# redmod-team/SympGPR

Measured on AMD Instinct MI355X. Metric: Gram-build GB/s + Cholesky fp64 TFLOP/s at N=65536 d=2; |alpha-alpha_ref|/|alpha_ref|, higher is better.
Workload: dtype f64

## Files before the change

include/sympgpr_probe.h:

```cpp
#ifndef SYMPGPR_PROBE_H
#define SYMPGPR_PROBE_H
#include <stddef.h>
#ifdef __cplusplus
extern "C" {
#endif

int sgpr_probe_mfma_f64(int waves_per_simd, int iters, double *tflops);
int sgpr_probe_hbm_write(size_t bytes, int reps, double *gbs);
int sgpr_probe_mfma_clock(int nacc, int waves_per_simd, int iters, double *out3);
int sgpr_probe_gemm(int m, int n, int k, int lower, double *out4);
int sgpr_probe_gemm_debug(int bits);
int sgpr_probe_leaf(double *out8);
int sgpr_probe_lat(double *out8);
int sgpr_probe_xcc(int nblocks, int *host_out);
int sgpr_probe_cumask(const unsigned *mask_words, int nwords, int nblocks, int *host_out);

int sgpr_probe_generated_eval(int family, int which, int m, const double *xa, const double *ya,
                              const double *xb, const double *yb, const double *l, int nl, double *out);

int sgpr_probe_queue_plan(int n, int nworkers, int *starts_out, int max_starts, unsigned *tasks_out, int max_tasks,
                          int *counts);
int sgpr_probe_queue_plan_partial(int n, int nworkers, int nq, int *starts_out, int max_starts, unsigned *tasks_out,
                                  int max_tasks, int *counts);
int sgpr_probe_queue_trace_begin(int max_tasks);
int sgpr_probe_queue_trace_end(unsigned long long *out, int max_tasks);
int sgpr_probe_queue_trace_clear(void);
int sgpr_probe_queue_postmortem(int always);
int sgpr_probe_queue_force_giveup(int on);
int sgpr_probe_tune(const char *name, double value);
int sgpr_probe_strassen_plan(int m, int n, int k, int lower, long smin, long kslab, long scratch_doubles, long long *out,
                             int max_records, int *count);
int sgpr_probe_gemm_strassen_dev(int m, int n, int k, double alpha, const double *A, size_t lda, const double *B, size_t ldb,
                                 double beta, double *C, size_t ldc, int lower, void *stream);
int sgpr_probe_gemm_nt2_dev(int m, int n, int k, double alpha, const double *A, size_t lda, const double *B, size_t ldb,
                            double beta, double *C, size_t ldc, double alpha2, double *C2, size_t ldc2, void *stream);
unsigned sgpr_probe_map_calls(void);
int sgpr_probe_map_team(int ntest, int n0);

int sgpr_probe_trsm_piece(int ticket, int cap, int strips, int out[5]);
int sgpr_probe_trsm_counts(int strips, int cap, unsigned long long out[2]);

int sgpr_probe_census(int na, int threads_a, int lds_a, int spin_a, const unsigned *mask_a, int nwords_a,
                      int nb, int threads_b, int lds_b, int spin_b, const unsigned *mask_b, int nwords_b,
                      unsigned long long *host_out);

#ifdef __cplusplus
}
#endif
#endif
```

sympgpr_amd/_lib.py:

```python
import ctypes as C
import os

import numpy as np

FAMILIES = {"A": 0, "B": 1, "C": 2, "D": 3, "USER": 4}
K_KERN, K_DXDX0, K_DYDY0, K_DXDY0 = 0, 1, 2, 3
K_DLX, K_DLY = 4, 8
K_DX, K_DY, K_DX0, K_DY0, K_DXDX0DY0, K_DYDY0DY0, K_DXDY0DY0 = 16, 17, 18, 19, 20, 21, 22
G_QQ, G_PQ, G_QP, G_PP, G_ALL, G_LOWER, G_OCML, G_DLX, G_DLY = 1, 2, 4, 8, 15, 16, 32, 64, 128
FIT_LOWER_ONLY, FIT_REG, FIT_BLOCK_QQ, FIT_BLOCK_PP = 1, 4, 8, 16
MAP_WRAP_Q, MAP_WRAP_P, MAP_EXPLICIT, MAP_LOSS_NEGP = 1, 2, 4, 8
E_ARG, E_NODEVICE, E_HIP, E_NOMEM, E_STATE = -1, -2, -3, -4, -5

ABI_VERSION = 5
_dp = C.POINTER(C.c_double)
_vp = C.c_void_p


class SympGPRError(RuntimeError):
    pass


class NoDeviceError(SympGPRError):
    pass


def lib_path():
    return os.path.join(os.path.dirname(os.path.abspath(__file__)), "lib", "libsympgpr_hip.so")


SIGNATURES = {
    "sgpr_abi_version": (C.c_int, []),
    "sgpr_last_error": (C.c_char_p, []),
    "sgpr_device_count": (C.c_int, []),
    "sgpr_set_device": (C.c_int, [C.c_int]),
    "sgpr_build_k_host": (C.c_int, [C.c_int, C.c_int, C.c_int, _dp, _dp, _dp, _dp, _dp, C.c_int, _dp, C.c_size_t]),
    "sgpr_buildkreg_host": (C.c_int, [C.c_int, C.c_int, C.c_int, _dp, _dp, _dp, _dp, _dp, C.c_int, _dp, C.c_size_t]),
    "sgpr_build_dk_host": (C.c_int, [C.c_int, C.c_int, C.c_int, C.c_int, _dp, _dp, _dp, _dp, _dp, C.c_int, _dp,
                                     C.c_size_t]),
    "sgpr_build_dkreg_host": (C.c_int, [C.c_int, C.c_int, C.c_int, C.c_int, _dp, _dp, _dp, _dp, _dp, C.c_int, _dp,
                                        C.c_size_t]),
    "sgpr_build_k_nd_host": (C.c_int, [C.c_int, C.c_int, C.c_int, C.c_int, _dp, C.c_size_t, _dp, C.c_size_t, _dp,
                                       C.c_int, _dp, C.c_size_t]),
    "sgpr_kernel_eval_host": (C.c_int, [C.c_int, C.c_int, C.c_int, _dp, _dp, _dp, _dp, _dp, C.c_int, _dp]),
    "sgpr_potrf_host": (C.c_int, [C.c_int, _dp, C.c_size_t]),
    "sgpr_potrs_host": (C.c_int, [C.c_int, _dp, C.c_size_t, _dp, C.c_size_t, C.c_int]),
    "sgpr_fit_create": (C.c_int, [C.c_int, C.c_int, _dp, _dp, _dp, _dp, C.c_int, C.c_double, C.c_uint, _vp,
                                  C.POINTER(_vp)]),
    "sgpr_fit_create_nd": (C.c_int, [C.c_int, C.c_int, C.c_int, _dp, C.c_size_t, _dp, _dp, C.c_int, C.c_double,
                                     C.c_uint, _vp, C.POINTER(_vp)]),
    "sgpr_fit_set_hyp": (C.c_int, [_vp, _dp, C.c_int, C.c_double]),
    "sgpr_fit_set_targets": (C.c_int, [_vp, _dp]),
    "sgpr_fit_build": (C.c_int, [_vp]),
    "sgpr_fit_factor": (C.c_int, [_vp]),
    "sgpr_fit_solve": (C.c_int, [_vp]),
    "sgpr_fit_run": (C.c_int, [_vp]),
    "sgpr_fit_alpha": (C.c_int, [_vp, _dp]),
    "sgpr_fit_nll": (C.c_int, [_vp, _dp]),
    "sgpr_fit_ldiag": (C.c_int, [_vp, _dp]),
    "sgpr_fit_get_matrix": (C.c_int, [_vp, _dp, C.c_size_t]),
    "sgpr_fit_solve_rhs": (C.c_int, [_vp, _dp, C.c_size_t, C.c_int]),
    "sgpr_fit_solve_rhs_dev": (C.c_int, [C.c_void_p, C.c_void_p, C.c_size_t, C.c_int]),
    "sgpr_fit_predict_rows": (C.c_int, [_vp, C.c_int, _dp, _dp, _dp, _dp]),
    "sgpr_fit_nll_grad": (C.c_int, [_vp, _dp]),
    "sgpr_fit_nll_grad_terms": (C.c_int, [_vp, _dp]),
    "sgpr_fit_eig": (C.c_int, [_vp, _dp, _dp]),
    "sgpr_syev_host": (C.c_int, [C.c_int, _dp, C.c_size_t, _dp]),
    "sgpr_fit_inverse": (C.c_int, [_vp, _dp, C.c_size_t]),
    "sgpr_fit_predict_nd": (C.c_int, [_vp, C.c_int, _dp, C.c_size_t, _dp]),
    "sgpr_fit_predict_cov": (C.c_int, [_vp, C.c_int, _dp, C.c_size_t, _dp, _dp]),
    "sgpr_fit_nll_grad_full": (C.c_int, [_vp, _dp, C.c_int]),
    "sgpr_fit_stage_ms": (C.c_int, [_vp, _dp, _dp, _dp]),
    "sgpr_fit_cond_estimate": (C.c_int, [_vp, C.c_int, _dp]),
    "sgpr_fit_trim": (C.c_int, [_vp]),
    "sgpr_fit_solve_rhs_ms": (C.c_int, [_vp, _dp]),
    "sgpr_potrf_info_dev": (C.c_int, [C.c_int, _vp]),
    "sgpr_trim": (C.c_int, []),
    "sgpr_fit_device_ptrs": (C.c_int, [_vp, C.POINTER(_vp), C.POINTER(C.c_size_t), C.POINTER(_vp)]),
    "sgpr_fit_destroy": (C.c_int, [_vp]),
    "sgpr_gram_pairs_dev": (C.c_int, [C.c_int, C.c_int, C.c_int, _vp, _vp, _vp, _vp, _dp, C.c_int, _vp, _vp, _vp,
                                      _vp, C.c_size_t, C.c_long, C.c_double, C.c_uint, _vp]),
    "sgpr_gram_nd_dev": (C.c_int, [C.c_int, C.c_int, C.c_int, C.c_int, _vp, C.c_size_t, _vp, C.c_size_t, _dp, C.c_int,
                                   _vp, C.c_size_t, C.c_size_t, C.c_size_t, C.c_long, C.c_double, _vp]),
    "sgpr_gram_reg_dev": (C.c_int, [C.c_int, C.c_int, C.c_int, _vp, _vp, _vp, _vp, _dp, C.c_int, _vp, C.c_size_t,
                                    C.c_long, C.c_double, _vp]),
    "sgpr_gram_nd_sel_dev": (C.c_int, [C.c_int, C.c_int, C.c_int, C.c_int, _vp, C.c_size_t, _vp, C.c_size_t, _dp, C.c_int,
                                       _vp, C.c_size_t, C.POINTER(C.c_long), C.POINTER(C.c_long), _vp]),
    "sgpr_potrf_workspace": (C.c_size_t, [C.c_int]),
    "sgpr_potrf_inverses_bytes": (C.c_size_t, [C.c_int]),
    "sgpr_release_device_streams": (C.c_int, [C.c_int]),
    "sgpr_family_has_p": (C.c_int, [C.c_int]),
    "sgpr_potrf_dev": (C.c_int, [C.c_int, _vp, C.c_size_t, _vp, C.c_size_t, _vp, _vp]),
    "sgpr_trsm_rlt_dev": (C.c_int, [C.c_int, C.c_int, _vp, C.c_size_t, _vp, C.c_size_t, _vp, _vp]),
    "sgpr_gemm_nt_dev": (C.c_int, [C.c_int, C.c_int, C.c_int, C.c_double, _vp, C.c_size_t, _vp, C.c_size_t,
                                   C.c_double, _vp, C.c_size_t, C.c_int, C.c_long, _vp]),
    "sgpr_profile_begin": (C.c_int, []),
    "sgpr_profile_end": (C.c_int, [_dp]),
    "sgpr_profile_launches": (C.c_int, [_dp, C.c_int]),
    "sgpr_gemm_nt_bc_dev": (C.c_int, [C.c_int, C.c_int, C.c_int, C.c_double, _vp, C.c_size_t, _vp, C.c_size_t,
                                      C.c_double, _vp, C.c_size_t, C.c_int, C.c_int, C.c_int, C.c_int, C.c_int, _vp]),
    "sgpr_trsv_dev": (C.c_int, [C.c_int, _vp, C.c_size_t, _vp, _vp, C.c_int, _vp]),
    "sgpr_gemv_sub_dev": (C.c_int, [C.c_int, C.c_int, C.c_int, _vp, C.c_size_t, _vp, _vp, _vp]),
    "sgpr_gemm_nn_dev": (C.c_int, [C.c_int, C.c_int, C.c_int, C.c_double, _vp, C.c_size_t, _vp, C.c_size_t, C.c_double, _vp,
                                   C.c_size_t, _vp]),
    "sgpr_trsm_rl_dev": (C.c_int, [C.c_int, C.c_int, _vp, C.c_size_t, _vp, C.c_size_t, _vp, _vp]),
    "sgpr_copy_blocks_dev": (C.c_int, [C.c_int, C.c_int, C.c_int, _vp, C.c_size_t, C.c_size_t, _vp, C.c_size_t, C.c_size_t, _vp]),
    "sgpr_predict_rows_dev": (C.c_int, [C.c_int, C.c_int, _vp, _vp, C.c_int, _vp, _vp, _dp, C.c_int, _vp, _vp, _vp,
                                        _vp]),
    "sgpr_predict_nd_dev": (C.c_int, [C.c_int, C.c_int, C.c_int, _vp, C.c_size_t, C.c_int, _vp, C.c_size_t, _dp, C.c_int,
                                      _vp, _vp, _vp]),
    "sgpr_predict_reg_dev": (C.c_int, [C.c_int, C.c_int, _vp, _vp, C.c_int, _vp, _vp, _dp, C.c_int, _vp, _vp, _vp]),
    "sgpr_applymap_host": (C.c_int, [C.c_int, C.c_int, C.c_int, C.c_int, _dp, C.c_int, C.c_int, _dp, _dp, _dp, _dp,
                                     C.c_int, C.c_int, _dp, _dp, _dp, _dp, _dp, _dp, _dp, _dp]),
    "sgpr_fit_applymap_nd": (C.c_int, [_vp, C.c_int, C.c_int, C.c_int, _dp, C.c_size_t, _dp, C.c_size_t, _dp, _dp,
                                       C.POINTER(C.c_int)]),
    "sgpr_applymap_nd_host": (C.c_int, [C.c_int, C.c_int, C.c_int, C.c_int, C.c_int, _dp, C.c_int, C.c_int, _dp, C.c_size_t,
                                        _dp, _dp, C.c_size_t, _dp, C.c_size_t, _dp, _dp, C.POINTER(C.c_int)]),
    "sgpr_potrs_vec_dev": (C.c_int, [C.c_int, _vp, C.c_size_t, _vp, _vp, _vp]),
    "sgpr_solve_status_dev": (C.c_int, [C.c_int, _vp, C.c_size_t, _vp, _vp]),
    "sgpr_fit_batch_max_order": (C.c_int, []),
    "sgpr_fit_batch": (C.c_int, [C.c_int, C.c_int, C.c_int, _dp, _dp, _dp, _dp, C.c_int, _dp, C.c_uint, _dp, _dp,
                                 C.POINTER(C.c_int)]),
    "sgpr_fit_batch_grad": (C.c_int, [C.c_int, C.c_int, C.c_int, _dp, _dp, _dp, _dp, C.c_int, _dp, C.c_uint, _dp, _dp, _dp,
                                      C.POINTER(C.c_int)]),
}

PROBE_SIGNATURES = {
    "sgpr_probe_mfma_f64": (C.c_int, [C.c_int, C.c_int, _dp]),
    "sgpr_probe_mfma_clock": (C.c_int, [C.c_int, C.c_int, C.c_int, _dp]),
    "sgpr_probe_gemm": (C.c_int, [C.c_int, C.c_int, C.c_int, C.c_int, _dp]),
    "sgpr_probe_gemm_debug": (C.c_int, [C.c_int]),
    "sgpr_probe_leaf": (C.c_int, [_dp]),
    "sgpr_probe_lat": (C.c_int, [_dp]),
    "sgpr_probe_cumask": (C.c_int, [C.POINTER(C.c_uint), C.c_int, C.c_int, C.POINTER(C.c_int)]),
    "sgpr_probe_xcc": (C.c_int, [C.c_int, C.POINTER(C.c_int)]),
    "sgpr_probe_hbm_write": (C.c_int, [C.c_size_t, C.c_int, _dp]),
    "sgpr_probe_generated_eval": (C.c_int, [C.c_int, C.c_int, C.c_int, _dp, _dp, _dp, _dp, _dp, C.c_int, _dp]),
    "sgpr_probe_queue_plan": (C.c_int, [C.c_int, C.c_int, C.POINTER(C.c_int), C.c_int, C.POINTER(C.c_uint), C.c_int,
                                        C.POINTER(C.c_int)]),
    "sgpr_probe_queue_plan_partial": (C.c_int, [C.c_int, C.c_int, C.c_int, C.POINTER(C.c_int), C.c_int, C.POINTER(C.c_uint),
                                                C.c_int, C.POINTER(C.c_int)]),
    "sgpr_probe_queue_trace_begin": (C.c_int, [C.c_int]),
    "sgpr_probe_queue_trace_end": (C.c_int, [C.POINTER(C.c_ulonglong), C.c_int]),
    "sgpr_probe_queue_postmortem": (C.c_int, [C.c_int]),
    "sgpr_probe_queue_force_giveup": (C.c_int, [C.c_int]),
    "sgpr_probe_tune": (C.c_int, [C.c_char_p, C.c_double]),
    "sgpr_probe_map_calls": (C.c_uint, []),
    "sgpr_probe_map_team": (C.c_int, [C.c_int, C.c_int]),
    "sgpr_probe_trsm_piece": (C.c_int, [C.c_int, C.c_int, C.c_int, C.POINTER(C.c_int)]),
    "sgpr_probe_trsm_counts": (C.c_int, [C.c_int, C.c_int, C.POINTER(C.c_ulonglong)]),
    "sgpr_probe_queue_trace_clear": (C.c_int, []),
    "sgpr_probe_strassen_plan": (C.c_int, [C.c_int, C.c_int, C.c_int, C.c_int, C.c_long, C.c_long, C.c_long,
                                           C.POINTER(C.c_longlong), C.c_int, C.POINTER(C.c_int)]),
    "sgpr_probe_gemm_strassen_dev": (C.c_int, [C.c_int, C.c_int, C.c_int, C.c_double, C.c_void_p, C.c_size_t, C.c_void_p, C.c_size_t,
                                               C.c_double, C.c_void_p, C.c_size_t, C.c_int, C.c_void_p]),
    "sgpr_probe_gemm_nt2_dev": (C.c_int, [C.c_int, C.c_int, C.c_int, C.c_double, C.c_void_p, C.c_size_t, C.c_void_p, C.c_size_t,
                                          C.c_double, C.c_void_p, C.c_size_t, C.c_double, C.c_void_p, C.c_size_t, C.c_void_p]),
    "sgpr_probe_census": (C.c_int, [C.c_int, C.c_int, C.c_int, C.c_int, C.POINTER(C.c_uint), C.c_int,
                                    C.c_int, C.c_int, C.c_int, C.c_int, C.POINTER(C.c_uint), C.c_int,
                                    C.POINTER(C.c_ulonglong)]),
}

_LIB = None
_PROBE = None


def load_library():
    global _LIB
    if _LIB is not None:
        return _LIB
    path = lib_path()
    if os.environ.get("SYMPGPR_NO_TORCH_PRELOAD") != "1":
        try:
            import torch
        except ImportError:
            pass
    if not os.path.exists(path):
        raise SympGPRError("%s is missing: run `python -c 'import __graft_entry__ as g; g.build()'` "
                           "(or make -C sympgpr_amd/csrc); there is no CPU fallback" % path)
    lib = C.CDLL(path)
    for name, (res, args) in SIGNATURES.items():
        fn = getattr(lib, name)
        fn.restype = res
        fn.argtypes = args
    if lib.sgpr_abi_version() != ABI_VERSION:
        raise SympGPRError("ABI version mismatch: %s is version %d, this package binds version %d -- rebuild it "
                           "(make -C sympgpr_amd/csrc)" % (path, lib.sgpr_abi_version(), ABI_VERSION))
    _LIB = lib
    import atexit
    atexit.register(_release_streams_at_exit)
    return lib


def _release_streams_at_exit():
    lib = _LIB
    if lib is None:
        return
    try:
        for dev in range(max(0, lib.sgpr_device_count())):
            lib.sgpr_release_device_streams(dev)
    except Exception:
        pass


def load_probe_library():
    global _PROBE
    if _PROBE is not None:
        return _PROBE
    load_library()
    path = os.path.join(os.path.dirname(lib_path()), "libsympgpr_probe.so")
    if not os.path.exists(path):
        raise SympGPRError("%s is missing: run make -C sympgpr_amd/csrc" % path)
    lib = C.CDLL(path)
    for name, (res, args) in PROBE_SIGNATURES.items():
        fn = getattr(lib, name)
        fn.restype = res
        fn.argtypes = args
    _PROBE = lib
    return lib


def device_count():
    return load_library().sgpr_device_count()


def check(rc, what=""):
    if rc == 0:
        return
    if rc > 0:
        raise np.linalg.LinAlgError("%d-th leading minor of the array is not positive definite" % rc)
    msg = load_library().sgpr_last_error().decode(errors="replace")
    if rc == E_NODEVICE:
        raise NoDeviceError(msg)
    raise SympGPRError("%s failed (%d): %s" % (what or "libsympgpr_hip call", rc, msg))


def dptr(a):
    return a.ctypes.data_as(_dp)


def f64(a):
    return np.ascontiguousarray(np.asarray(a, dtype=np.float64))


def family_has_p(fam):
    return bool(load_library().sgpr_family_has_p(family_id(fam)))


def family_id(fam):
    if isinstance(fam, str):
        return FAMILIES[fam]
    return int(fam)
```

sympgpr_amd/csrc/chol.hip:

```cpp
#include <algorithm>
#include <cstdlib>
#include <mutex>
#include <vector>

#include "cholq.h"
#include "common.h"
#include "gemm_tile.h"
#include "leaf.h"

namespace sgpr {

namespace {

using namespace leaf;


__global__ __launch_bounds__(LT) void leaf_kernel(int nb, double *A, size_t lda, double *inv,
                                                  int *dinfo, int goff, int mode,
                                                  unsigned long long *stamps)
{
    __shared__ double s[LEAF_LDS];
    if (nb == LEAF) leaf_body(s, (int)LEAF, A, lda, inv, dinfo, goff, mode, stamps);
    else            leaf_body(s, nb, A, lda, inv, dinfo, goff, mode, stamps);
}
// ... 1138 lines not shown
void release_all_streams_at_exit()
{
    int ndev = 0;
    if (hipGetDeviceCount(&ndev) != hipSuccess) { (void)hipGetLastError(); return; }
    for (int dev = 0; dev < ndev && dev < 64; ++dev) {
        hipStream_t drop[9] = {};
        int nd = 0;
        {
            std::lock_guard<std::mutex> lock(g_side_mu);
            if (g_side[dev]) { drop[nd++] = g_side[dev]; g_side[dev] = nullptr; }
        }
        {
            QueueDevice &qd = g_qdev[dev];
            std::lock_guard<std::mutex> lock(qd.mu);
            for (int r = 0; r < 4; ++r) {
                if (qd.workers[r]) { drop[nd++] = qd.workers[r]; qd.workers[r] = nullptr; }
                if (qd.panels[r]) { drop[nd++] = qd.panels[r]; qd.panels[r] = nullptr; }
            }
            qd.failed = true;
        }
        if (!nd) continue;
        int cur = -1;
        (void)hipGetDevice(&cur);
        if (cur != dev) (void)hipSetDevice(dev);
        for (int q = 0; q < nd; ++q) (void)hipStreamDestroy(drop[q]);
        if (cur != dev && cur >= 0) (void)hipSetDevice(cur);
    }
    (void)hipGetLastError();
}

int release_streams(int dev)
{
    {
        bool any = false;
        {
            std::lock_guard<std::mutex> lock(g_side_mu);
            any = g_side[dev] != nullptr;
        }
        QueueDevice &qd = g_qdev[dev];
        std::lock_guard<std::mutex> lock(qd.mu);
        for (int r = 0; r < 4; ++r) any = any || qd.workers[r] || qd.panels[r];
        any = any || qd.done;
        if (!any) return 0;
    }
    int cur = -1;
    SGPR_HIP(hipGetDevice(&cur));
    if (cur != dev) SGPR_HIP(hipSetDevice(dev));
    hipError_t first = hipSuccess;
    auto drop = [&](hipStream_t &s) {
        if (!s) return;
        hipError_t e = hipStreamSynchronize(s);
        if (e == hipSuccess) e = hipStreamDestroy(s);
        if (e != hipSuccess && first == hipSuccess) first = e;
        s = nullptr;
    };
    {
        std::lock_guard<std::mutex> lock(g_side_mu);
        drop(g_side[dev]);
    }
    {
        QueueDevice &qd = g_qdev[dev];
        std::lock_guard<std::mutex> lock(qd.mu);
        for (int r = 0; r < 4; ++r) { drop(qd.workers[r]); drop(qd.panels[r]); }
        if (qd.done) {
            const hipError_t e = hipEventDestroy(qd.done);
            if (e != hipSuccess && first == hipSuccess) first = e;
            qd.done = nullptr;
        }
        qd.ncu = 0;
        qd.failed = false;
        for (int r = 0; r < 4; ++r) qd.overlap_ok[r] = false;
    }
    if (cur != dev) (void)hipSetDevice(cur);
    SGPR_HIP(first);
    return 0;
}

int potrf_lookahead(int n, double *A, size_t lda, const Ctx &c, int nb, int off0)
{
    if (nb == 0 && c.qws && c.flags && cholq::eligible(n) && (lda & 1) == 0 && (((uintptr_t)A & 15) == 0) && off0 % LEAF == 0) {
        const int rq = potrf_queue(n, A, lda, c, off0);
        if (rq <= 0) return rq;
    }
    hipStream_t sp = nullptr;
    {
        int dev = -1;
        const int rc0 = side_stream(c.st, &sp, &dev);
        if (rc0) return rc0;
    }
    static const int pmode = (int)tune("la_panel", 3);
    const bool fused_cap = pmode == 3 && c.flags && n % LEAF == 0 && (lda & 1) == 0 && (((uintptr_t)A & 15) == 0) &&
                           off0 % LEAF == 0;
    std::vector<int> starts;
    {
        static const int t0_env = (int)tune("la_t0", 0);
        const int t0 = t0_env > 0 ? t0_env : (n >= 24576 ? 12288 : 1 << 30);
        static const int t1 = (int)tune("la_t1", 6144);
        static const int t2 = (int)tune("la_t2", 2048);
        for (int pos = 0; pos < n;) {
            starts.push_back(pos);
            const int rem = n - pos;
            int w = nb > 0 ? nb : (rem > t0 ? 2048 : (rem > t1 ? 1024 : (rem > t2 ? 512 : 256)));
            if (nb == 0 && !fused_cap) w = la_block(n);
            pos += std::min(w, rem);
        }
        starts.push_back(n);
    }
    const int nblk = (int)starts.size() - 1;
    int wmax = 0;
    for (int k = 0; k < nblk; ++k) wmax = std::max(wmax, starts[k + 1] - starts[k]);
    EventSet es;
    {
        const int rc0 = es.create(3 * (size_t)nblk + 3);
        if (rc0) return rc0;
    }
    std::vector<hipEvent_t> &ev = es.ev;
    const hipStream_t su = c.st;
    Ctx cp{c.inv, c.dinfo, sp, 0, c.flags};
    const bool fused_ok = fused_cap && wmax % LEAF == 0 && wmax / LEAF <= PW_MAX;
    const bool left = pmode != 2, right_in = pmode == 0 || pmode == 3;
    auto panel = [&](int k) -> int {
        const int k0 = starts[k], w = starts[k + 1] - k0, rows = n - k0, below = rows - w;
        double *Akk = A + k0 + (size_t)k0 * lda;
        if (fused_ok) {
            PanelArgs pa{};
            pa.P = Akk; pa.lda = lda;
            pa.R = rows / LEAF; pa.W = w / LEAF;
            const int nbelow = pa.R - pa.W;
            const double m_u2 = (double)(rows + w);
            const double u2_us = k > 0 ? m_u2 * m_u2 * (starts[k] - starts[k - 1]) / 55e6 : 0.0;
            static const double split_ratio = tune("panel_split_ratio", 3.0);
            const bool split = nbelow > 0 && k > 0 && u2_us > split_ratio * (125.0 * pa.W + 100.0);
            if (split) {
                pa.R = pa.W;
                pa.G = pa.W;
            } else {
                const double strip_us = 30.0 * (pa.W * (pa.W + 1) / 2 + pa.W), chain_us = 125.0 * pa.W;
                int per_wg = (int)((0.7 * u2_us - 0.5 * chain_us) / strip_us);
                per_wg = std::max(1, std::min(per_wg, 4));
                const int nwg = std::min((nbelow + per_wg - 1) / per_wg, PANEL_G_MAX - pa.W);
                pa.G = pa.W + (nbelow > 0 ? std::max(1, nwg) : 0);
            }
            static const bool helpers_on = tune("panel_helpers", 1) != 0, below_early_on = tune("panel_below_early", 1) != 0;
            pa.NH = helpers_on && pa.W > 2 ? (pa.W - 1) * (pa.W - 2) / 2 : 0;
            if (pa.G + pa.NH > PANEL_G_MAX) pa.NH = 0;
            pa.below_early = below_early_on ? 1 : 0;
            static const bool tiles_on = tune("panel_tiles", 1) != 0;
            static const double tile_mult = tune("panel_tile_mult", 1.0);
            if (tiles_on && !split && nbelow > 0 && pa.W >= 2 && nbelow < PFLAG_STRIDE) {
                const double chain_us = 60.0 * pa.W + 50.0;
                int nt = u2_us < chain_us ? nbelow * pa.W : (int)(tile_mult * (pa.G - pa.W));
                nt = std::max(1, std::min(std::min(nt, nbelow * pa.W), PANEL_G_MAX - pa.W - pa.NH));
                pa.tiles = 1;
                pa.G = pa.W + nt;
            }
            const int t0 = (off0 + k0) / LEAF;
            pa.inv = cp.inv + (size_t)t0 * LEAF * LEAF;
            pa.dinfo = cp.dinfo; pa.goff = off0 + k0;
            pa.flags = c.flags + (size_t)t0 * PFLAG_STRIDE;
            pa.dbg = (PANEL_DBG && g_panel_dbg) ? g_panel_dbg + (size_t)16 * t0 : nullptr;
            hipLaunchKernelGGL(panel_kernel, dim3(std::max(pa.G + pa.NH, 8 * (pa.W - 1) + 1)), dim3(LT), 0, sp, pa);
            SGPR_CHECK_LAUNCH();
            if (split) return trsm_rec(below, w, Akk, lda, Akk + w, lda, off0 + k0, cp);
            return 0;
        }
        if (!left) {
            int rc = potrf_rec(w, Akk, lda, off0 + k0, cp);
            if (rc) return rc;
            if (below > 0) rc = trsm_rec(below, w, Akk, lda, Akk + w, lda, off0 + k0, cp);
            return rc;
        }
        for (int c0 = 0; c0 < w; c0 += LEAF) {
            const int nj = std::min((int)LEAF, w - c0), mrows = rows - c0;
            double *Pj = Akk + c0 + (size_t)c0 * lda;
            int rc;
            if (!right_in && c0 > 0 &&
                (rc = gemm_nt(mrows, nj, c0, -1.0, Akk + c0, lda, Akk + c0, lda, 1.0, Pj, lda, 0, 0, sp)))
                return rc;
            double *invj = cp.inv + (size_t)((off0 + k0 + c0) / LEAF) * LEAF * LEAF;
            hipLaunchKernelGGL(leaf_kernel, dim3(1), dim3(LT), 0, sp, nj, Pj, lda, invj, cp.dinfo, off0 + k0 + c0,
                               (int)LEAF_FACTOR, (unsigned long long *)nullptr);
            SGPR_CHECK_LAUNCH();
            if (mrows > nj && (rc = gemm_nt(mrows - nj, nj, nj, 1.0, Pj + nj, lda, invj, LEAF, 0.0, Pj + nj, lda, 0, 0, sp)))
                return rc;
            const int ncols = w - c0 - nj;
            if (right_in && ncols > 0 &&
                (rc = gemm_nt(mrows - nj, ncols, nj, -1.0, Pj + nj, lda, Pj + nj, lda, 1.0, Pj + nj + (size_t)nj * lda, lda, 1, 0, sp)))
                return rc;
        }
        return 0;
    };
    int rc;
    SGPR_HIP(hipEventRecord(ev[2 * nblk], su));
    SGPR_HIP(hipStreamWaitEvent(sp, ev[2 * nblk], 0));
    StreamJoin join{sp, su, ev[2 * nblk + 1]};
    gemm_set_overlap(1);
    if ((rc = panel(0))) return rc;
    SGPR_HIP(hipEventRecord(ev[0], sp));
    for (int k = 0; k < nblk; ++k) {
        const int k0 = starts[k], w = starts[k + 1] - k0;
        const int k1 = k0 + w;
        if (k1 >= n) break;
        const int w1 = starts[k + 2] - k1, k2 = k1 + w1;
        const double *Lk = A + (size_t)k0 * lda;
        if (k > 0) SGPR_HIP(hipStreamWaitEvent(sp, ev[2 * (k - 1) + 1], 0));
        if ((rc = gemm_nt(n - k1, w1, w, -1.0, Lk + k1, lda, Lk + k1, lda, 1.0, A + k1 + (size_t)k1 * lda, lda, 1, 0, sp)))
            return rc;
        const double u2_us = (double)(n - k2) * (n - k2) * w / 55e6;
        const bool chain_bound = u2_us < 1.5 * (125.0 * (w1 / LEAF) + 100.0);
        if (chain_bound) SGPR_HIP(hipEventRecord(ev[2 * nblk + 2 + k], sp));
        if ((rc = panel(k + 1))) return rc;
        SGPR_HIP(hipEventRecord(ev[2 * (k + 1)], sp));
        SGPR_HIP(hipStreamWaitEvent(su, chain_bound ? ev[2 * nblk + 2 + k] : ev[2 * k], 0));
        if (k2 < n &&
            (rc = gemm_nt(n - k2, n - k2, w, -1.0, Lk + k2, lda, Lk + k2, lda, 1.0, A + k2 + (size_t)k2 * lda, lda, 1, 0, su)))
            return rc;
        SGPR_HIP(hipEventRecord(ev[2 * k + 1], su));
    }
    return 0;
}

}

size_t potrf_batch_flag_bytes(int nbatch) { return ((size_t)nbatch * PFLAG_STRIDE + 1) * sizeof(int); }
int potrf_batch_max_order() { return PW_MAX * (int)LEAF; }

int potrf_batch(int nbatch, int npad, double *A, size_t stride_a, size_t lda, double *inv, size_t stride_inv, int *flags,
                int *info, hipStream_t st)
{
    if (nbatch < 0 || npad <= 0 || npad % LEAF != 0 || npad > PW_MAX * (int)LEAF || lda < (size_t)npad || (lda & 1) != 0 ||
        ((uintptr_t)A & 15) != 0 || (stride_a & 1) != 0) {
        set_error("potrf_batch: bad order / leading dimension / alignment");
        return SGPR_E_ARG;
    }
    if (nbatch == 0) return 0;
    SGPR_HIP(hipMemsetAsync(info, 0, (size_t)nbatch * sizeof(int), st));
    return potrf_batch_panel(nbatch, npad, 0, npad / (int)LEAF, A, stride_a, lda, inv, stride_inv, flags, info, st);
}

int potrf_batch_panel(int nbatch, int npad, int k0, int Wd, double *A, size_t stride_a, size_t lda, double *inv, size_t stride_inv,
                      int *flags, int *info, hipStream_t st)
{
    const int R = (npad - k0) / (int)LEAF;
    if (nbatch <= 0 || k0 < 0 || k0 % LEAF != 0 || Wd < 1 || Wd > PW_MAX || Wd > R || R > PANEL_G_MAX) {
        set_error("potrf_batch_panel: bad panel");
        return SGPR_E_ARG;
    }
    SGPR_HIP(hipMemsetAsync(flags, 0, potrf_batch_flag_bytes(nbatch), st));
    const int below_max = (int)tune("batch_below", 0);
    const int below = R - Wd <= 0 ? 0 : (below_max > 0 && below_max < R - Wd ? below_max : R - Wd);
    PanelBatch q{A, stride_a, lda, inv, stride_inv, flags, info, flags + (size_t)nbatch * PFLAG_STRIDE, Wd, nbatch, R, k0, Wd + below};
    hipLaunchKernelGGL(panel_batch_kernel, dim3((unsigned)(nbatch * (Wd + below))), dim3(LT), 0, st, q);
    SGPR_CHECK_LAUNCH();
    return 0;
}

bool potrf_queue_mark_failed(hipStream_t st)
{
    const bool used = t_last_potrf_used_queue;
    if (!used) return false;
    int dev = -1;
    if ((st ? hipStreamGetDevice(st, &dev) : hipGetDevice(&dev)) != hipSuccess || dev < 0 || dev >= 64) { (void)hipGetLastError(); return false; }
    QueueDevice &qd = g_qdev[dev];
    std::lock_guard<std::mutex> lock(qd.mu);
    qd.failed = true;
    return true;
}

int potrf_trim()
{
    for (int dev = 0; dev < 64; ++dev) {
        EventPool &p = t_event_pool[dev];
        if (p.ev.empty() || p.top != 0) continue;
        for (hipEvent_t e : p.ev) (void)hipEventDestroy(e);
        p.ev.clear();
    }
    (void)hipGetLastError();
    return strassen_trim();
}

int release_device_streams(int dev)
{
    if (dev < 0 || dev >= 64) { set_error("release_device_streams: device index out of range"); return SGPR_E_ARG; }
    return release_streams(dev);
}

int potrf(int n, double *A, size_t lda, void *work, size_t lwork, int *dinfo, hipStream_t st)
{
    if (n < 0 || (n > 0 && lda < (size_t)n)) { set_error("potrf: bad n / lda"); return SGPR_E_ARG; }
    if (lwork < potrf_workspace(n)) { set_error("potrf: workspace too small"); return SGPR_E_ARG; }
    SGPR_HIP(hipMemsetAsync(dinfo, 0, sizeof(int), st));
    if (n == 0) return 0;
    int *flags = reinterpret_cast<int *>(static_cast<char *>(work) + inv_bytes(n));
    SGPR_HIP(hipMemsetAsync(flags, 0, flag_bytes(n), st));
    static const int mode = [] { const char *e = getenv("SGPR_POTRF"); return !e ? 0 : (e[0] == 'r' ? 1 : 2); }();
    static const int nb_env = [] { const char *e = getenv("SGPR_POTRF_NB"); return e ? atoi(e) : 0; }();
    static const int la_max_env = [] { const char *e = getenv("SGPR_LA_MAX"); return (int)tune("la_max", e ? atoi(e) : 57344); }();
    t_last_potrf_used_queue = false;
    Ctx c{static_cast<double *>(work), dinfo, st, mode == 1 ? 0 : la_max_env, flags};
    if (cholq::ws_bytes(n) > 0) c.qws = static_cast<char *>(work) + inv_bytes(n) + flag_bytes(n) + pub_bytes(n);
    c.strassen = true;
    if (n > c.la_max && n > LEAF) {
        const int n1 = split(n), n2 = n - n1, n11 = split(n1);
        strassen_reserve(std::max(strassen_scratch_doubles(n2, n2, n1, 1), strassen_scratch_doubles(n2, n1 - n11, n11, 0)), st);
    }
    const bool dbg = PANEL_DBG && getenv("SGPR_PANEL_DBG") != nullptr;
    const int T = (n + LEAF - 1) / LEAF;
    if (dbg) {
        (void)hipMalloc((void **)&g_panel_dbg, sizeof(unsigned long long) * 16 * T);
        (void)hipMemset(g_panel_dbg, 0, sizeof(unsigned long long) * 16 * T);
    }
    int rc;
    if (mode == 2 || (nb_env > 0 && mode == 0 && n > 4 * LEAF && n <= c.la_max))
        rc = potrf_lookahead(n, A, lda, c, nb_env > 0 ? nb_env : 0, 0);
    else
        rc = potrf_rec(n, A, lda, 0, c);
    if (dbg) {
        (void)hipStreamSynchronize(st);
        std::vector<unsigned long long> h(16 * (size_t)T);
        (void)hipMemcpy(h.data(), g_panel_dbg, h.size() * 8, hipMemcpyDeviceToHost);
        (void)hipFree(g_panel_dbg);
        g_panel_dbg = nullptr;
        std::vector<double> d[9];
        for (int t = 1; t + 1 < T; ++t) {
            const unsigned long long *p = &h[16 * t], *q = &h[16 * (t + 1)];
            if (!p[0] || !p[5] || !q[0]) continue;
            d[0].push_back((p[1] - p[0]) * 0.01);
            d[1].push_back((p[2] - p[1]) * 0.01);
            d[2].push_back((p[3] - p[2]) * 0.01);
            d[3].push_back((p[4] - p[3]) * 0.01);
            d[4].push_back(((double)q[0] - (double)p[4]) * 0.01);
            d[5].push_back((p[5] - p[4]) * 0.01);
            d[3].back() = ((double)p[4] - (double)p[1]) * 0.01;
            d[1].back() = (p[6] - p[0]) * 0.01;
            d[2].back() = (p[7] - p[6]) * 0.01;
            d[6].push_back((p[11] - p[4]) * 0.01);
            d[7].push_back((p[12] - p[11]) * 0.01);
            d[8].push_back(((double)q[2] - (double)p[4]) * 0.01);
            if (getenv("SGPR_PANEL_DBG_ALL"))
                fprintf(stderr, "  col %3d: leaf entry -> factor %.1f -> flag %.1f | next strip at wait %.1f, saw E %.1f | its solve %.1f, update %.1f\n", t,
                        (p[11] - p[4]) * 0.01, (p[12] - p[4]) * 0.01, ((double)q[2] - (double)p[4]) * 0.01, ((double)q[0] - (double)p[4]) * 0.01,
                        (q[1] - q[0]) * 0.01, ((double)q[4] - (double)q[1]) * 0.01);
        }
        auto med = [](std::vector<double> &x) { std::sort(x.begin(), x.end()); return x.empty() ? 0.0 : x[x.size() / 2]; };
        fprintf(stderr, "panel chain n=%d (%zu columns): E seen -> solve stored %.1f | E seen -> staged %.1f | -> MFMA part done %.1f | (solve stored -> leaf entry %.1f) | "
                "leaf entry -> next E seen %.1f (factor %.1f, -> flag set %.1f; next strip at its wait %.1f) | whole leaf %.1f us\n", n, d[0].size(), med(d[0]), med(d[1]), med(d[2]), med(d[3]), med(d[4]),
                med(d[6]), med(d[7]), med(d[8]), med(d[5]));
    }
    return rc;
}

int trsm_rlt(int m, int n, const double *L, size_t ldl, double *B, size_t ldb, const void *work,
             hipStream_t st)
{
    if (m <= 0 || n <= 0) return 0;
    Ctx c{const_cast<double *>(static_cast<const double *>(work)), nullptr, st};
    return trsm_rec(m, n, L, ldl, B, ldb, 0, c);
}

static bool use_strips(int n, const double *L, size_t ldl)
{
    static const bool off = [] { const char *e = getenv("SGPR_TRSV"); return e && e[0] == 'r'; }();
    return !off && n > TRSV_BLOCK && trsv_strips_ok(n, L, ldl);
}
static int *solve_state(int n, const void *work)
{
    return reinterpret_cast<int *>(const_cast<char *>(static_cast<const char *>(work)) + inv_bytes(n));
}
static double *solve_pub(int n, const void *work)
{
    return reinterpret_cast<double *>(const_cast<char *>(static_cast<const char *>(work)) + inv_bytes(n) + flag_bytes(n));
}

bool trsv_uses_strips(int n, const double *L, size_t ldl) { return use_strips(n, L, ldl); }

int solve_status(int n, const double *L, size_t ldl, const void *work, hipStream_t st)
{
    if (n <= 0 || !use_strips(n, L, ldl)) { SGPR_HIP(hipStreamSynchronize(st)); return 0; }
    int h[8] = {};
    SGPR_HIP(hipMemcpyAsync(h, solve_state(n, work), sizeof(h), hipMemcpyDeviceToHost, st));
    SGPR_HIP(hipStreamSynchronize(st));
    if (h[2] || h[6]) { set_error("triangular solve: a hand-off between strips timed out"); return SGPR_E_HIP; }
    return 0;
}
const int *trsv_state(int n, const void *work) { return solve_state(n, work); }

int potrs_vec(int n, const double *L, size_t ldl, void *work, double *b, hipStream_t st)
{
    if (n <= 0) return 0;
    Ctx c{const_cast<double *>(static_cast<const double *>(work)), nullptr, st};
    if (use_strips(n, L, ldl)) {
        int *state = solve_state(n, work);
        double *pub = solve_pub(n, work);
        SGPR_HIP(hipMemsetAsync(state, 0, 8 * sizeof(int), st));
        SGPR_HIP(hipMemsetAsync(pub, 0xFF, (size_t)2 * n * sizeof(double), st));
        int rc = trsv_strips(n, L, ldl, c.inv, b, 0, state, pub, st);
        if (rc) return rc;
        return trsv_strips(n, L, ldl, c.inv, b, 1, state + 4, pub + n, st);
    }
    int rc = trsv_n_rec(n, L, ldl, b, 0, c);
    if (rc) return rc;
    return trsv_t_rec(n, L, ldl, b, 0, c);
}

int trsm_rl(int m, int n, const double *L, size_t ldl, double *B, size_t ldb, const void *work, hipStream_t st)
{
    if (m <= 0 || n <= 0) return 0;
    Ctx c{const_cast<double *>(static_cast<const double *>(work)), nullptr, st};
    return trsm_rl_rec(m, n, L, ldl, B, ldb, 0, c);
}

int trsm_rlt_off(int m, int n, const double *L, size_t ldl, double *B, size_t ldb, const void *work, int off, hipStream_t st)
{
    if (m <= 0 || n <= 0) return 0;
    if (off < 0 || off % (int)LEAF) { set_error("trsm_rlt_off: offset not on a leaf boundary"); return SGPR_E_ARG; }
    Ctx c{const_cast<double *>(static_cast<const double *>(work)), nullptr, st};
    return trsm_rec(m, n, L, ldl, B, ldb, off, c);
}
int trsm_rl_off(int m, int n, const double *L, size_t ldl, double *B, size_t ldb, const void *work, int off, hipStream_t st)
{
    if (m <= 0 || n <= 0) return 0;
    if (off < 0 || off % (int)LEAF) { set_error("trsm_rl_off: offset not on a leaf boundary"); return SGPR_E_ARG; }
    Ctx c{const_cast<double *>(static_cast<const double *>(work)), nullptr, st};
    return trsm_rl_rec(m, n, L, ldl, B, ldb, off, c);
}

bool potrs_mat_uses_strips(int n, int nrhs, const double *L, size_t ldl)
{
    return nrhs >= 2 && nrhs <= 256 && use_strips(n, L, ldl) && trsm_strips_ok(n, L, ldl);
}
size_t potrs_mat_scratch(int n, int nrhs, const double *L, size_t ldl)
{
    if (n <= 0 || nrhs <= 0) return 8;
    return potrs_mat_uses_strips(n, nrhs, L, ldl) ? trsm_strips_scratch(n) : (size_t)n * nrhs * sizeof(double);
}

int potrs_mat(int n, const double *L, size_t ldl, const void *work, double *B, size_t ldb, int nrhs,
              double *scratch, hipStream_t st)
{
    if (n <= 0 || nrhs <= 0) return 0;
    if (potrs_mat_uses_strips(n, nrhs, L, ldl))
        return potrs_strips(n, L, ldl, static_cast<const double *>(work), B, ldb, nrhs, solve_state(n, work), scratch, st);
    int rc = transpose(n, nrhs, B, ldb, scratch, (size_t)nrhs, st);
    if (rc) return rc;
    if ((rc = trsm_rlt(nrhs, n, L, ldl, scratch, (size_t)nrhs, work, st))) return rc;
    if ((rc = trsm_rl(nrhs, n, L, ldl, scratch, (size_t)nrhs, work, st))) return rc;
    return transpose(nrhs, n, scratch, (size_t)nrhs, B, ldb, st);
}

int potrs_mat_fwd(int n, const double *L, size_t ldl, const void *work, double *B, size_t ldb, int nrhs,
                  double *scratch, hipStream_t st)
{
    if (n <= 0 || nrhs <= 0) return 0;
    if (potrs_mat_uses_strips(n, nrhs, L, ldl))
        return trsm_strips_fwd(n, L, ldl, static_cast<const double *>(work), B, ldb, nrhs, solve_state(n, work), scratch, st);
    int rc = transpose(n, nrhs, B, ldb, scratch, (size_t)nrhs, st);
    if (rc) return rc;
    if ((rc = trsm_rlt(nrhs, n, L, ldl, scratch, (size_t)nrhs, work, st))) return rc;
    return transpose(nrhs, n, scratch, (size_t)nrhs, B, ldb, st);
}

int trsv(int n, const double *L, size_t ldl, void *work, double *b, int trans, hipStream_t st)
{
    if (n <= 0) return 0;
    Ctx c{const_cast<double *>(static_cast<const double *>(work)), nullptr, st};
    if (use_strips(n, L, ldl)) {
        int *state = solve_state(n, work);
        double *pub = solve_pub(n, work);
        SGPR_HIP(hipMemsetAsync(state, 0, 4 * sizeof(int), st));
        SGPR_HIP(hipMemsetAsync(pub, 0xFF, (size_t)n * sizeof(double), st));
        return trsv_strips(n, L, ldl, c.inv, b, trans, state, pub, st);
    }
    return trans ? trsv_t_rec(n, L, ldl, b, 0, c) : trsv_n_rec(n, L, ldl, b, 0, c);
}

int leaf_probe(double *A, size_t lda, double *inv, int *dinfo, unsigned long long *stamps, hipStream_t st)
{
    hipLaunchKernelGGL(leaf_kernel, dim3(1), dim3(LT), 0, st, (int)LEAF, A, lda, inv, dinfo, 0, (int)LEAF_FACTOR, stamps);
    SGPR_CHECK_LAUNCH();
    return 0;
}

int leaf_inverses(int n, const double *L, size_t ldl, void *work, int *dinfo, hipStream_t st)
{
    if (n <= 0) return 0;
    Ctx c{static_cast<double *>(work), dinfo, st};
    return leaves_invert_only(n, const_cast<double *>(L), ldl, c);
}

}
```

sympgpr_amd/csrc/common.h:

```cpp
#pragma once
#include <hip/hip_runtime.h>
#include <cstddef>
#include <cstdint>
#include <string>
#include <vector>

#include "../../include/sympgpr_hip.h"

namespace sgpr {

void set_error(const std::string &msg);
double tune(const char *name, double dflt);
void tune_set(const char *name, double v);
int hip_fail(hipError_t e, const char *what, const char *file, int line);

#define SGPR_HIP(call)                                                          \
    do {                                                                        \
        hipError_t e__ = (call);                                                \
        if (e__ != hipSuccess) return ::sgpr::hip_fail(e__, #call, __FILE__, __LINE__); \
    } while (0)

#define SGPR_CHECK_LAUNCH() SGPR_HIP(hipGetLastError())

struct KConst {
    double lx, ly, p, sig;
    double lx2, ly2;
    double inv_lx2, inv_ly2;
    double cxx, cyy, cxy;
    double hscale;
    double inv_lx, inv_ly, inv_lx3, inv_ly3;
    double gxx;
};
enum { DERIV_NONE = 0, DERIV_LX = 1, DERIV_LY = 2 };
int make_kconst(int family, const double *hyp, int nhyp, KConst *out);
bool family_has_p(int family);
int make_kconst_l(int family, const double *l, int nl, KConst *out);

int gram_pairs(int family, int mi, int mj, const double *xb, const double *yb, const double *xa,
               const double *ya, const KConst &kc, double *qq, double *Pq, double *qP, double *PP,
               size_t ld, long diag_off, double noise, unsigned flags, hipStream_t st);
int gram_reg(int family, int mi, int mj, const double *xb, const double *yb, const double *xa,
             const double *ya, const KConst &kc, double *G, size_t ld, long diag_off, double noise,
             hipStream_t st, int deriv = DERIV_NONE);
int kernel_eval(int family, int which, int m, const double *xa, const double *ya, const double *xb,
                const double *yb, const KConst &kc, double *out, hipStream_t st);
int predict_rows(int family, int m, const double *q, const double *P, int n0, const double *xtr,
                 const double *ytr, const KConst &kc, const double *alpha, double *out_p,
                 double *out_q, hipStream_t st);
int predict_reg(int family, int m, const double *q, const double *P, int n0, const double *xtr,
                const double *ytr, const KConst &kc, const double *alpha, double *out,
                hipStream_t st);

int applymap_team(int ntest, int n0);
size_t applymap_team_ws(int ntest, int n0);
int applymap(int family, int mode, int nm, int ntest, int n0, const double *xtr, const double *ytr,
             const KConst &kc, const double *alpha, int n0p, const double *xtrp, const double *ytrp,
             const KConst &kcp, const double *alphap, const double *Q0, const double *P0, double *qmap,
             double *pmap, double *pdiff, void *team_ws, hipStream_t st);
int applymap_status(const void *team_ws, int ntest, int n0);
unsigned applymap_last_calls();

int gram_nd(int family, int d, int mi, int mj, const double *Xb, size_t ldxb, const double *Xa, size_t ldxa,
            const double *hyp, int nhyp, double *K, size_t ld, size_t rstride, size_t cstride, long diag_off,
            double noise, hipStream_t st);
int gram_nd_sel(int family, int d, int mi, int mj, const double *Xb, size_t ldxb, const double *Xa, size_t ldxa,
                const double *hyp, int nhyp, double *K, size_t ld, const long *roff, const long *coff, hipStream_t st);
int predict_nd(int family, int d, int m, const double *Xt, size_t ldxt, int n0, const double *Xtr, size_t ldxtr,
               const double *hyp, int nhyp, const double *alpha, double *out, hipStream_t st);
int applymap_nd(int family, int d, int mode, int nm, int ntest, int n0, const double *Xtr, size_t ldxtr, const double *hyp,
                int nhyp, const double *alpha, const double *Q0, const double *P0, double *qmap, double *pmap, int *iters,
                hipStream_t st);

int gemm_nt(int m, int n, int k, double alpha, const double *A, size_t lda, const double *B,
            size_t ldb, double beta, double *C, size_t ldc, int lower, long diag_off,
            hipStream_t st);
int gemm_nt_bc(int m, int n, int k, double alpha, const double *A, size_t lda, const double *B,
               size_t ldb, double beta, double *C, size_t ldc, int lower, const int *bc5,
               hipStream_t st);
int gemm_nn(int m, int n, int k, double alpha, const double *A, size_t lda, const double *B, size_t ldb,
            double beta, double *C, size_t ldc, hipStream_t st);
int gemm_nt_two(int m, int n, int k, double alpha, const double *A, size_t lda, const double *B, size_t ldb, double beta,
             double *C, size_t ldc, double alpha2, double *C2, size_t ldc2, hipStream_t st);
constexpr int STRASSEN_REC = 16;
enum { PLAN_SUM = 1, PLAN_PROD = 2, PLAN_CLASSIC = 3 };
int gemm_nt_strassen(int m, int n, int k, double alpha, const double *A, size_t lda, const double *B, size_t ldb, double beta,
                     double *C, size_t ldc, int lower, hipStream_t st);
int strassen_plan(int m, int n, int k, int lower, long smin, long kslab, size_t scratch_doubles, std::vector<long long> &out);
size_t strassen_scratch_doubles(int m, int n, int k, int lower);
void strassen_reserve(size_t doubles, hipStream_t st);
int strassen_trim();
int gemm_profile_begin();
int gemm_profile_end(double *out12);
int gemm_profile_launches(double *buf, int max_records);
void gemm_set_overlap(int on);
int gemm_nt_diag(int m, int n, int k, double alpha, const double *A, size_t lda, const double *B, size_t ldb,
                 double beta, double *C, size_t ldc, int lower, unsigned long long *stamps, int dbg, hipStream_t st);

constexpr int LEAF = 128;
constexpr int POTRF_HANDOFF_TIMEOUT = -1000001;
constexpr int SOLVE_HANDOFF_TIMEOUT = -1000002;
inline int info_status(int info)
{
    if (info >= 0) return info;
    set_error(info == POTRF_HANDOFF_TIMEOUT ? "potrf: a hand-off inside the panel kernel timed out"
              : info == SOLVE_HANDOFF_TIMEOUT ? "solve: a hand-off between the strips of a triangular solve timed out" : "potrf: internal error");
    return SGPR_E_HIP;
}
size_t potrf_workspace(int n);
int potrf(int n, double *A, size_t lda, void *work, size_t lwork, int *dinfo, hipStream_t st);
size_t potrf_batch_flag_bytes(int nbatch);
int potrf_batch_max_order();
int potrf_batch(int nbatch, int npad, double *A, size_t stride_a, size_t lda, double *inv, size_t stride_inv, int *flags,
                int *info, hipStream_t st);
int potrf_batch_panel(int nbatch, int npad, int k0, int Wd, double *A, size_t stride_a, size_t lda, double *inv, size_t stride_inv,
                      int *flags, int *info, hipStream_t st);
bool potrf_queue_mark_failed(hipStream_t st);
int release_device_streams(int dev);
int trsm_rlt(int m, int n, const double *L, size_t ldl, double *B, size_t ldb, const void *work,
             hipStream_t st);
int potrs_vec(int n, const double *L, size_t ldl, void *work, double *b, hipStream_t st);
int solve_status(int n, const double *L, size_t ldl, const void *work, hipStream_t st);
int trsm_rl(int m, int n, const double *L, size_t ldl, double *B, size_t ldb, const void *work, hipStream_t st);
int trsm_rlt_off(int m, int n, const double *L, size_t ldl, double *B, size_t ldb, const void *work, int off, hipStream_t st);
int trsm_rl_off(int m, int n, const double *L, size_t ldl, double *B, size_t ldb, const void *work, int off, hipStream_t st);
int potrs_mat(int n, const double *L, size_t ldl, const void *work, double *B, size_t ldb, int nrhs, double *scratch,
              hipStream_t st);
int potrs_mat_fwd(int n, const double *L, size_t ldl, const void *work, double *B, size_t ldb, int nrhs, double *scratch,
                  hipStream_t st);
size_t potrs_mat_scratch(int n, int nrhs, const double *L, size_t ldl);
bool potrs_mat_uses_strips(int n, int nrhs, const double *L, size_t ldl);
int trsv(int n, const double *L, size_t ldl, void *work, double *b, int trans, hipStream_t st);
bool trsv_uses_strips(int n, const double *L, size_t ldl);
const int *trsv_state(int n, const void *work);
int leaf_probe(double *A, size_t lda, double *inv, int *dinfo, unsigned long long *stamps, hipStream_t st);
int leaf_inverses(int n, const double *L, size_t ldl, void *work, int *dinfo, hipStream_t st);

bool trsv_strips_ok(int n, const double *L, size_t ldl);
int trsv_strips(int n, const double *L, size_t ldl, const double *inv, double *b, int trans, int *state ,
                double *pub , hipStream_t st);
int trsv_strips_batch(int nbatch, int n, const double *L, size_t sL, size_t ldl, const double *inv, size_t sInv, double *b, size_t sB,
                      int trans, int *state, int sState, double *pub, hipStream_t st);

constexpr int TRSM_YLD = 80;
constexpr int TRSM_FOLD = 5;
constexpr int TRSM_STATE_INTS = 16;
bool trsm_strips_ok(int n, const double *L, size_t ldl);
void trsm_piece_of(int u, int C, int T, int out[5]);
void trsm_piece_counts(int T, int C, size_t out[2]);
size_t trsm_strips_scratch(int n);
int potrs_strips(int n, const double *L, size_t ldl, const double *inv, double *B, size_t ldb, int nrhs, int *state ,
                 double *scratch, hipStream_t st);
int trsm_strips_fwd(int n, const double *L, size_t ldl, const double *inv, double *B, size_t ldb, int nrhs, int *state,
                    double *scratch, hipStream_t st);

constexpr int POSTCOV_COLS = 256;
size_t postcov_partial_doubles(int n, int D, int mc);
int postcov(int D, int n, int mc, const double *V, size_t ldv, const double *Kss, size_t ldk, double *part, double *cov,
            hipStream_t st);

size_t nll_grad_full_scratch(int n, int N, int nacc);
int nll_grad_full(int family, int d, bool reg, int N, int n, const double *L, size_t ldl, const void *work, const double *X,
                  const double *alpha, const double *l, const double *pp, int nacc, double *scratch, double *out,
                  hipStream_t st);

int fit_batch_max_order();
int fit_batch_trim();
int potrf_trim();
int fit_batch(int family, int nbatch, int npts, const double *x, const double *y, const double *z, const double *hyp,
              int nhyp, const double *sig2n, unsigned flags, double *alpha, double *nll, int *info);
int fit_batch_grad_max_order();
int fit_batch_grad(int family, int nbatch, int npts, const double *x, const double *y, const double *z, const double *hyp,
                   int nhyp, const double *sig2n, unsigned flags, double *alpha, double *nll, double *grad, int *info);

int zero_strict_upper(int n, double *A, size_t lda, hipStream_t st);
int sym_fill_upper(int n, double *A, size_t lda, hipStream_t st);
int nll_reduce(int n, const double *L, size_t ldl, const double *z, const double *alpha,
               double *dout , hipStream_t st);
int copy_diag(int n, const double *A, size_t lda, double *d, hipStream_t st);
int dot(int n, const double *a, const double *b, double *out, hipStream_t st);
constexpr int SUMSQ_SCRATCH = 1024;
int syev_jacobi(int n, double *A, size_t lda, double *V, size_t ldv, double *w_host, int max_sweeps,
                int *sweeps_done, hipStream_t st);
int sumsq(size_t count, const double *a, double *part, double *out, hipStream_t st);
int trace(int n, const double *A, size_t lda, double *out, hipStream_t st);
int transpose(int m, int n, const double *A, size_t lda, double *B, size_t ldb, hipStream_t st);
int gemv_n_sub(int m, int k, const double *A, size_t lda, const double *x, double *y,
               hipStream_t st);
int gemv_t_sub(int m, int k, const double *A, size_t lda, const double *x, double *y,
               hipStream_t st);

}
```

sympgpr_amd/csrc/gemm_f64.hip:

```cpp
#include <algorithm>
#include <atomic>
#include <cstdlib>
#include <mutex>
#include <type_traits>
#include <vector>

#include "common.h"
#include "gemm_tile.h"

namespace sgpr {

namespace {

struct ProfRec { double flop; int big; int m, n, k, lower, overlap; };
struct Prof {
    std::mutex mu;
    std::atomic<bool> on{false};
    std::vector<hipEvent_t> pool;
    std::vector<ProfRec> recs;
    long dropped = 0;
};
constexpr int PROF_POOL = 8192;
Prof g_prof;
thread_local int t_overlap = 0;

using namespace tile;

template <int BM, int BN>
__global__ __launch_bounds__(64 * (BM / 64) * (BN / 64), (BM >= 128 ? 2 : 1)) void gemm_nt_kernel(const GemmArgs g)
{
    constexpr int LDA_S = BM + PAD, LDB_S = BN + PAD;
    constexpr int STAGES = (BM == 256 && BN == 128) ? SGPR_GEMM_STAGES : 2;
    __shared__ double smem[STAGES * BK * (LDA_S + LDB_S)];
    int tile_r, tile_c;
    if (!tile_of<(SR * BM) / (4 * BN)>(g, tile_r, tile_c)) return;
    const int row0 = tile_r * BM, col0 = tile_c * BN;
    if (g.lower) {
        const long rb = ((long)min(row0 + BM, g.m) - 1) / g.lblk, cb = (long)col0 / g.lblk;
        if (rb * g.lpr + g.lpi < cb * g.lpc + g.lpj) return;
    }
    const bool aligned = ((((uintptr_t)g.A | (uintptr_t)g.B) & 15) == 0) && (((g.lda | g.ldb) & 1) == 0);
    const bool fast = aligned && (row0 + BM <= g.m) && (col0 + BN <= g.n) && (g.k % BK == 0);
    if (g.transb) {
        if (fast) gemm_body<BM, BN, true, true>(g, smem, tile_r, tile_c);
        else      gemm_body<BM, BN, false, true>(g, smem, tile_r, tile_c);
        return;
    }
    if constexpr (BM % 128 == 0) {
        if (fast && !(g.dbg & 16)) { gemm_body_dma<BM, BN, STAGES>(g, smem, tile_r, tile_c); return; }
    }
    if (fast) gemm_body<BM, BN, true>(g, smem, tile_r, tile_c);
    else      gemm_body<BM, BN, false>(g, smem, tile_r, tile_c);
}

__global__ __launch_bounds__(512, 2) void gemm_nt2_kernel(const GemmArgs g)
{
    constexpr int BM = 256, BN = 128, LDA_S = BM + PAD, LDB_S = BN + PAD;
    __shared__ double smem[SGPR_GEMM_STAGES * BK * (LDA_S + LDB_S)];
    int tile_r, tile_c;
    if (!tile_of<(SR * BM) / (4 * BN)>(g, tile_r, tile_c)) return;
    const int row0 = tile_r * BM, col0 = tile_c * BN;
    const bool aligned = ((((uintptr_t)g.A | (uintptr_t)g.B) & 15) == 0) && (((g.lda | g.ldb) & 1) == 0);
    const bool fast = aligned && (row0 + BM <= g.m) && (col0 + BN <= g.n) && (g.k % BK == 0);
    if (fast) gemm_body_dma<BM, BN, SGPR_GEMM_STAGES, true>(g, smem, tile_r, tile_c);
    else      gemm_body<BM, BN, false, false, true>(g, smem, tile_r, tile_c);
}

__global__ __launch_bounds__(256) void block_sum_kernel(int rows, int cols, const double *X, size_t ldx, const double *Y, size_t ldy,
                                                        double sign, double *T)
{
    const int nrc = (rows + 511) / 512, ncg = (cols + 3) / 4;
    const long pieces = (long)nrc * ncg;
    for (long p = blockIdx.x; p < pieces; p += gridDim.x) {
        const int cg = (int)(p / nrc), rc = (int)(p - (long)cg * nrc);
        const int r = rc * 512 + 2 * (int)threadIdx.x;
        if (r >= rows) continue;
        double2_t x[4], y[4];
#pragma unroll
        for (int u = 0; u < 4; ++u) {
            const int c = min(cg * 4 + u, cols - 1);
            x[u] = *reinterpret_cast<const double2_t *>(X + (size_t)r + (size_t)c * ldx);
            y[u] = *reinterpret_cast<const double2_t *>(Y + (size_t)r + (size_t)c * ldy);
        }
#pragma unroll
        for (int u = 0; u < 4; ++u) {
            const int c = cg * 4 + u;
            if (c < cols) *reinterpret_cast<double2_t *>(T + (size_t)r + (size_t)c * (size_t)rows) = x[u] + sign * y[u];
        }
    }
}

}

int gemm_nt(int m, int n, int k, double alpha, const double *A, size_t lda, const double *B,
            size_t ldb, double beta, double *C, size_t ldc, int lower, long diag_off,
            hipStream_t st)
{
    const int bc[5] = {1, 1, (int)diag_off, 1, 0};
    return gemm_nt_bc(m, n, k, alpha, A, lda, B, ldb, beta, C, ldc, lower, bc, st);
}

static int gemm_launch(int m, int n, int k, double alpha, const double *A, size_t lda, const double *B,
                       size_t ldb, double beta, double *C, size_t ldc, int lower, const int *bc, int transb,
                       hipStream_t st, unsigned long long *stamps = nullptr, int dbg = 0, double *C2 = nullptr,
                       size_t ldc2 = 0, double alpha2 = 0.0);

static int gemm_chunked(int m, int n, int k, double alpha, const double *A, size_t lda, const double *B,
                        size_t ldb, double beta, double *C, size_t ldc, int lower, const int *bc,
                        hipStream_t st, double *C2, size_t ldc2, double alpha2)
{
    static const int kmax = [] { const char *e = getenv("SGPR_GEMM_KMAX"); return e ? atoi(e) : 8192; }();
    if (kmax >= 128 && k > kmax) {
        const int nchunk = (k + kmax - 1) / kmax;
        const int step = ((k + nchunk - 1) / nchunk + 127) / 128 * 128;
        for (int k0 = 0; k0 < k; k0 += step) {
            const int rc = gemm_launch(m, n, std::min(step, k - k0), alpha, A + (size_t)k0 * lda, lda, B + (size_t)k0 * ldb, ldb,
                                       k0 == 0 ? beta : 1.0, C, ldc, lower, bc, 0, st, nullptr, 0, C2, ldc2, alpha2);
            if (rc) return rc;
        }
        return 0;
    }
    return gemm_launch(m, n, k, alpha, A, lda, B, ldb, beta, C, ldc, lower, bc, 0, st, nullptr, 0, C2, ldc2, alpha2);
}

int gemm_nt_bc(int m, int n, int k, double alpha, const double *A, size_t lda, const double *B,
               size_t ldb, double beta, double *C, size_t ldc, int lower, const int *bc,
               hipStream_t st)
{
    return gemm_chunked(m, n, k, alpha, A, lda, B, ldb, beta, C, ldc, lower, bc, st, nullptr, 0, 0.0);
}

int gemm_nt_two(int m, int n, int k, double alpha, const double *A, size_t lda, const double *B, size_t ldb, double beta,
             double *C, size_t ldc, double alpha2, double *C2, size_t ldc2, hipStream_t st)
{
    const int bc[5] = {1, 1, 0, 1, 0};
    if (!C2) { set_error("gemm_nt_two: null second destination"); return SGPR_E_ARG; }
    return gemm_chunked(m, n, k, alpha, A, lda, B, ldb, beta, C, ldc, 0, bc, st, C2, ldc2, alpha2);
}

static int gemm_launch(int m, int n, int k, double alpha, const double *A, size_t lda, const double *B,
                       size_t ldb, double beta, double *C, size_t ldc, int lower, const int *bc, int transb,
                       hipStream_t st, unsigned long long *stamps, int dbg, double *C2, size_t ldc2, double alpha2)
{
    const bool plain = bc[0] == 1 && bc[1] == 1 && bc[3] == 1 && bc[4] == 0;
    const long diag_off = plain ? bc[2] : 1;
    if (bc[0] < 1 || bc[1] < 1 || bc[3] < 1) { set_error("gemm_nt: bad block-cyclic descriptor"); return SGPR_E_ARG; }
    if (m < 0 || n < 0 || k < 0) { set_error("gemm_nt: negative extent"); return SGPR_E_ARG; }
    if (m == 0 || n == 0) return 0;
    if (lda < (size_t)m || ldb < (size_t)(transb ? k : n) || ldc < (size_t)m) {
        set_error("gemm: leading dimension too small");
        return SGPR_E_ARG;
    }
    if (C2 && (lower || transb || ldc2 < (size_t)m)) { set_error("gemm: bad second destination"); return SGPR_E_ARG; }
    GemmArgs g{m, n, k, alpha, beta, A, lda, B, ldb, C, ldc, lower, diag_off, transb, stamps, 0, 0, 0, 0, 0, 0,
               0, 0, bc[0], bc[1], bc[2], bc[3], bc[4], dbg, nullptr, C2, ldc2, alpha2};
    auto set_map = [&](int bm, int bn) {
        g.tiles_m = (m + bm - 1) / bm;
        g.tiles_n = (n + bn - 1) / bn;
        const int SC = (SR * bm) / (4 * bn);
        g.n_sr = (g.tiles_m + SR - 1) / SR;
        g.n_sc = (g.tiles_n + SC - 1) / SC;
        g.tri = (lower && diag_off == 0 && m == n) ? 1 : 0;
        if (g.tri) {
            long full = 0;
            for (int sc = 0; sc < g.n_sc; ++sc) full += std::max(g.n_sr - sc / 4 - 1, 0);
            g.n_full = (int)full;
            g.n_grp = (g.n_sc + 3) / 4;
            g.n_super = g.n_full + 4 * g.n_grp;
        }
        if (!g.tri) g.n_super = g.n_sr * g.n_sc;
        return (unsigned)(((g.n_super + 7) / 8) * 8 * SR * SC);
    };
    int slot = -1;
    ProfRec rec{};
    if (g_prof.on.load(std::memory_order_acquire)) {
        std::lock_guard<std::mutex> lock(g_prof.mu);
        if (g_prof.on.load(std::memory_order_relaxed)) {
            if ((int)g_prof.recs.size() < PROF_POOL) {
                double elems = (double)m * n;
                if (lower && plain) {
                    elems = 0.0;
                    for (int j = 0; j < n; ++j) {
                        long first = (long)j - diag_off;
                        if (first < 0) first = 0;
                        if (first < m) elems += (double)(m - first);
                    }
                } else if (lower) {
                    elems = 0.0;
                    const long blk = bc[0];
                    for (long j = 0; j < n; ++j) {
                        const long cbg = (j / blk) * bc[3] + bc[4], jo = j % blk;
                        for (long rb = 0; rb * blk < m; ++rb) {
                            const long rbg = rb * bc[1] + bc[2], rows = std::min(blk, (long)m - rb * blk);
                            if (rbg > cbg) elems += (double)rows;
                            else if (rbg == cbg) elems += (double)std::max(0L, rows - jo);
                        }
                    }
                }
                rec.flop = 2.0 * k * elems;
                rec.m = m; rec.n = n; rec.k = k; rec.lower = lower; rec.overlap = t_overlap;
                slot = (int)g_prof.recs.size();
                g_prof.recs.push_back(rec);
            } else {
                ++g_prof.dropped;
            }
        }
    }
    if (slot >= 0) SGPR_HIP(hipEventRecord(g_prof.pool[2 * slot], st));
    const long big = (long)((m + 255) / 256) * ((n + 127) / 128);
    static const bool prefer_big = tune("gemm_small_tile", 0) == 0;
    static const double small_mb = tune("gemm_small_mb", 0.0);
    const double op_bytes = 8.0 * (double)k * ((A == B && lda == ldb) ? (double)std::max(m, n) : (double)m + n);
    const bool small_k = op_bytes <= small_mb * 1e6 && m > 128 && n > 128;
    if (C2) {
        const dim3 grid(set_map(256, 128));
        hipLaunchKernelGGL(gemm_nt2_kernel, grid, dim3(512), 0, st, g);
        rec.big = 1;
    } else if (n <= 128 && m <= 32768 && !(dbg & 8)) {
        const dim3 grid(set_map(64, 128));
        hipLaunchKernelGGL((gemm_nt_kernel<64, 128>), grid, dim3(128), 0, st, g);
    } else if (prefer_big && !(dbg & 8) && !small_k && (big >= 256 || (m >= 256 && n == 128))) {
        const dim3 grid(set_map(256, 128));
        hipLaunchKernelGGL((gemm_nt_kernel<256, 128>), grid, dim3(512), 0, st, g);
        rec.big = 1;
    } else {
        const dim3 grid(set_map(128, 128));
        hipLaunchKernelGGL((gemm_nt_kernel<128, 128>), grid, dim3(256), 0, st, g);
    }
    SGPR_CHECK_LAUNCH();
    if (slot >= 0) {
        SGPR_HIP(hipEventRecord(g_prof.pool[2 * slot + 1], st));
        if (rec.big) {
            std::lock_guard<std::mutex> lock(g_prof.mu);
            if (slot < (int)g_prof.recs.size()) g_prof.recs[slot].big = 1;
        }
    }
    return 0;
}

int gemm_nt_diag(int m, int n, int k, double alpha, const double *A, size_t lda, const double *B, size_t ldb,
                 double beta, double *C, size_t ldc, int lower, unsigned long long *stamps, int dbg, hipStream_t st)
{
    const int bc[5] = {1, 1, 0, 1, 0};
    return gemm_launch(m, n, k, alpha, A, lda, B, ldb, beta, C, ldc, lower, bc, 0, st, stamps, dbg);
}

int gemm_nn(int m, int n, int k, double alpha, const double *A, size_t lda, const double *B, size_t ldb,
            double beta, double *C, size_t ldc, hipStream_t st)
{
    const int bc[5] = {1, 1, 0, 1, 0};
    return gemm_launch(m, n, k, alpha, A, lda, B, ldb, beta, C, ldc, 0, bc, 1, st);
}

void gemm_set_overlap(int on) { t_overlap = on; }

int gemm_profile_begin()
{
    std::lock_guard<std::mutex> lock(g_prof.mu);
    if (g_prof.pool.empty()) {
        g_prof.pool.resize(2 * (size_t)PROF_POOL);
        for (size_t i = 0; i < g_prof.pool.size(); ++i) {
            const hipError_t e = hipEventCreate(&g_prof.pool[i]);
            if (e != hipSuccess) {
                for (size_t j = 0; j < i; ++j) (void)hipEventDestroy(g_prof.pool[j]);
                g_prof.pool.clear();
                return hip_fail(e, "hipEventCreate (profile pool)", __FILE__, __LINE__);
            }
        }
        g_prof.recs.reserve(PROF_POOL);
    }
    g_prof.recs.clear();
    g_prof.dropped = 0;
    g_prof.on = true;
    return 0;
}

static std::vector<double> g_last_launches;
int gemm_profile_launches(double *buf, int max_records)
{
    std::lock_guard<std::mutex> lock(g_prof.mu);
    const int n = (int)(g_last_launches.size() / 7);
    if (buf)
        for (int i = 0; i < n && i < max_records; ++i)
            for (int j = 0; j < 7; ++j) buf[7 * i + j] = g_last_launches[7 * i + j];
    return n;
}

int gemm_profile_end(double *out)
{
    std::lock_guard<std::mutex> lock(g_prof.mu);
    g_prof.on = false;
    g_last_launches.clear();
    for (int i = 0; i < 12; ++i) out[i] = 0.0;
    out[11] = (double)g_prof.dropped;
    for (size_t i = 0; i < g_prof.recs.size(); ++i) {
        const ProfRec &r = g_prof.recs[i];
        SGPR_HIP(hipEventSynchronize(g_prof.pool[2 * i + 1]));
        float ms = 0.f;
        SGPR_HIP(hipEventElapsedTime(&ms, g_prof.pool[2 * i], g_prof.pool[2 * i + 1]));
        const int o = r.big ? (r.overlap ? 8 : 0) : 3;
        out[o] += 1.0; out[o + 1] += r.flop; out[o + 2] += ms;
        if (r.flop > out[6]) { out[6] = r.flop; out[7] = ms; }
        for (double v : {(double)r.m, (double)r.n, (double)r.k, (double)r.lower, (double)r.big, (double)ms, (double)r.overlap})
            g_last_launches.push_back(v);
    }
    g_prof.recs.clear();
    return 0;
}

namespace {
struct PlanCfg {
    long smin;
    long kslab;
    size_t scratch;
};
void put(std::vector<long long> &out, std::initializer_list<long long> v)
{
    size_t i = 0;
    for (long long x : v) { out.push_back(x); ++i; }
    for (; i < STRASSEN_REC; ++i) out.push_back(0);
}
long slab_of(long k, const PlanCfg &c)
{
    if (k <= 0 || k % 32 != 0 || c.kslab < 32) return 0;
    const long nslab = (k + c.kslab - 1) / c.kslab;
    const long step = ((k + nslab - 1) / nslab + 31) / 32 * 32;
    const long kmin = std::max(c.smin / 2, 16L);
    const long last = k - (nslab - 1) * step;
    if (last <= 0 || step / 2 < kmin || last / 2 < kmin) return 0;
    return step;
}
bool qualifies(long m, long n, long k, const PlanCfg &c)
{
    if (m <= 0 || n <= 0 || m % 512 != 0 || n % 256 != 0) return false;
    if (m / 2 < c.smin || n / 2 < c.smin) return false;
    const long step = slab_of(k, c);
    if (!step) return false;
    return (size_t)(m / 2 + n / 2) * (size_t)(step / 2) <= c.scratch;
}
void plan_gemm(long m, long n, long k, long ar, long br, long cr, long cc, const PlanCfg &c, std::vector<long long> &out)
{
    if (!qualifies(m, n, k, c)) {
        put(out, {PLAN_CLASSIC, 0, ar, 0, br, 0, m, n, k, cr, cc});
        return;
    }
    const long m2 = m / 2, n2 = n / 2, step = slab_of(k, c);
    for (long k0 = 0; k0 < k; k0 += step) {
        const long k2 = std::min(step, k - k0) / 2;
        const long a1 = ar, a2 = ar + m2, b1 = br, b2 = br + n2, j1 = k0, j2 = k0 + k2;
        const long c1r = cr, c2r = cr + m2, c1c = cc, c2c = cc + n2;
        auto sum = [&](int side, long xr, long xc, long yr, long yc, int sign) {
            put(out, {PLAN_SUM, side, side ? n2 : m2, k2, xr, xc, yr, yc, sign});
        };
        auto prod = [&](int as, long pr, long pc, int bs, long qr, long qc, long d1r, long d1c, int s1, long d2r, long d2c, int s2) {
            put(out, {PLAN_PROD, as, pr, pc, bs, qr, qc, m2, n2, k2, d1r, d1c, s1, d2r, d2c, s2});
        };
        sum(0, a1, j1, a2, j2, +1); sum(1, b1, j1, b2, j2, +1);
        prod(1, 0, 0, 1, 0, 0, c1r, c1c, +1, c2r, c2c, +1);
        sum(0, a2, j1, a2, j2, +1);
        prod(1, 0, 0, 0, b1, j1, c2r, c1c, +1, c2r, c2c, -1);
        sum(1, b2, j1, b2, j2, -1);
        prod(0, a1, j1, 1, 0, 0, c1r, c2c, +1, c2r, c2c, +1);
        sum(1, b1, j2, b1, j1, -1);
        prod(0, a2, j2, 1, 0, 0, c1r, c1c, +1, c2r, c1c, +1);
        sum(0, a1, j1, a1, j2, +1);
        prod(1, 0, 0, 0, b2, j2, c1r, c1c, -1, c1r, c2c, +1);
        sum(0, a2, j1, a1, j1, -1); sum(1, b1, j1, b2, j1, +1);
        prod(1, 0, 0, 1, 0, 0, c2r, c2c, +1, 0, 0, 0);
        sum(0, a1, j2, a2, j2, -1); sum(1, b1, j2, b2, j2, +1);
        prod(1, 0, 0, 1, 0, 0, c1r, c1c, +1, 0, 0, 0);
    }
}
void plan_syrk(long n, long k, long r0, const PlanCfg &c, std::vector<long long> &out)
{
    const long h = n / 2;
    if (n % 2 != 0 || !qualifies(h, h, k, c)) {
        put(out, {PLAN_CLASSIC, 1, r0, 0, r0, 0, n, n, k, r0, r0});
        return;
    }
    plan_syrk(h, k, r0, c, out);
    plan_gemm(h, h, k, r0 + h, r0, r0 + h, r0, c, out);
    plan_syrk(h, k, r0 + h, c, out);
}
size_t plan_need(const std::vector<long long> &plan)
{
    size_t need[2] = {0, 0};
    for (size_t i = 0; i + STRASSEN_REC <= plan.size(); i += STRASSEN_REC)
        if (plan[i] == PLAN_SUM) need[plan[i + 1]] = std::max(need[plan[i + 1]], (size_t)plan[i + 2] * (size_t)plan[i + 3]);
    return need[0] + need[1];
}

bool strassen_on()
{
    static const bool on = [] { const char *e = getenv("SGPR_GEMM_STRASSEN"); return !(e && e[0] == '0'); }();
    return on;
}
PlanCfg default_cfg()
{
    static const long smin = std::max(128L, (long)tune("gemm_strassen_min", 8192));
    static const long kslab = std::max(32L, (long)tune("gemm_strassen_kslab", 16384));
    return PlanCfg{smin, kslab, ~(size_t)0};
}

struct Scratch {
    std::mutex mu;
    double *p = nullptr;
    size_t cap = 0, failed = 0;
    hipEvent_t ev = nullptr;
    hipStream_t last = nullptr;
    bool used = false;
};
Scratch g_scratch[64];

bool scratch_ensure(Scratch &s, size_t need)
{
    static const bool forced_fail = tune("gemm_strassen_noscratch", 0) != 0;
    if (forced_fail) return false;
    if (s.cap >= need) return true;
    if (s.failed && need >= s.failed) return false;
    if (s.p) { (void)hipFree(s.p); s.p = nullptr; s.cap = 0; s.used = false; }
    if (hipMalloc((void **)&s.p, need * sizeof(double)) != hipSuccess) {
        (void)hipGetLastError();
        s.p = nullptr;
        s.failed = need;
        return false;
    }
    s.cap = need;
    return true;
}
int device_of(hipStream_t st)
{
    int dev = -1;
    if ((st ? hipStreamGetDevice(st, &dev) : hipGetDevice(&dev)) != hipSuccess) { (void)hipGetLastError(); return -1; }
    return (dev >= 0 && dev < 64) ? dev : -1;
}

int block_sum(int rows, int cols, const double *X, size_t ldx, const double *Y, size_t ldy, double sign, double *T, hipStream_t st)
{
    const long pieces = (long)((rows + 511) / 512) * ((cols + 3) / 4);
    hipLaunchKernelGGL(block_sum_kernel, dim3((unsigned)std::min(pieces, 2048L)), dim3(256), 0, st, rows, cols, X, ldx, Y, ldy, sign, T);
    SGPR_CHECK_LAUNCH();
    return 0;
}

int run_plan(const std::vector<long long> &plan, double alpha, const double *A, size_t lda, const double *B, size_t ldb,
             double beta, double *C, size_t ldc, double *SA, double *SB, hipStream_t st)
{
    for (size_t i = 0; i + STRASSEN_REC <= plan.size(); i += STRASSEN_REC) {
        const long long *r = &plan[i];
        int rc = 0;
        if (r[0] == PLAN_SUM) {
            const double *P = r[1] ? B : A;
            const size_t ld = r[1] ? ldb : lda;
            rc = block_sum((int)r[2], (int)r[3], P + r[4] + (size_t)r[5] * ld, ld, P + r[6] + (size_t)r[7] * ld, ld, (double)r[8],
                           r[1] ? SB : SA, st);
        } else if (r[0] == PLAN_PROD) {
            const int m = (int)r[7], n = (int)r[8], k = (int)r[9];
            const double *Ap = r[1] ? SA : A + r[2] + (size_t)r[3] * lda;
            const double *Bp = r[4] ? SB : B + r[5] + (size_t)r[6] * ldb;
            double *C1 = C + r[10] + (size_t)r[11] * ldc;
            if (r[15]) rc = gemm_nt_two(m, n, k, alpha * (double)r[12], Ap, r[1] ? (size_t)m : lda, Bp, r[4] ? (size_t)n : ldb, 1.0, C1, ldc,
                                     alpha * (double)r[15], C + r[13] + (size_t)r[14] * ldc, ldc, st);
            else       rc = gemm_nt(m, n, k, alpha * (double)r[12], Ap, r[1] ? (size_t)m : lda, Bp, r[4] ? (size_t)n : ldb, 1.0, C1, ldc, 0, 0, st);
        } else {
            rc = gemm_nt((int)r[6], (int)r[7], (int)r[8], alpha, A + r[2] + (size_t)r[3] * lda, lda, B + r[4] + (size_t)r[5] * ldb, ldb,
                         beta, C + r[9] + (size_t)r[10] * ldc, ldc, (int)r[1], 0, st);
        }
        if (rc) return rc;
    }
    return 0;
}
}

int strassen_plan(int m, int n, int k, int lower, long smin, long kslab, size_t scratch_doubles, std::vector<long long> &out)
{
    if (m < 0 || n < 0 || k < 0 || (lower && m != n)) { set_error("strassen_plan: bad extents"); return SGPR_E_ARG; }
    PlanCfg c = default_cfg();
    if (smin >= 0) c.smin = std::max(128L, smin);
    if (kslab >= 0) c.kslab = std::max(32L, kslab);
    c.scratch = scratch_doubles;
    out.clear();
    if (lower) plan_syrk(n, k, 0, c, out);
    else       plan_gemm(m, n, k, 0, 0, 0, 0, c, out);
    return 0;
}

size_t strassen_scratch_doubles(int m, int n, int k, int lower)
{
    std::vector<long long> plan;
    if (!strassen_on() || strassen_plan(m, n, k, lower, -1, -1, ~(size_t)0, plan)) return 0;
    return plan_need(plan);
}

void strassen_reserve(size_t doubles, hipStream_t st)
{
    const int dev = device_of(st);
    if (!doubles || dev < 0 || !strassen_on()) return;
    Scratch &s = g_scratch[dev];
    std::lock_guard<std::mutex> lock(s.mu);
    (void)scratch_ensure(s, doubles);
}

int strassen_trim()
{
    for (Scratch &s : g_scratch) {
        std::lock_guard<std::mutex> lock(s.mu);
        if (s.p) (void)hipFree(s.p);
        if (s.ev) (void)hipEventDestroy(s.ev);
        s.p = nullptr; s.ev = nullptr; s.cap = 0; s.failed = 0; s.used = false; s.last = nullptr;
    }
    (void)hipGetLastError();
    return 0;
}

int gemm_nt_strassen(int m, int n, int k, double alpha, const double *A, size_t lda, const double *B, size_t ldb, double beta,
                     double *C, size_t ldc, int lower, hipStream_t st)
{
    const bool aligned = ((((uintptr_t)A | (uintptr_t)B) & 15) == 0) && (((lda | ldb) & 1) == 0);
    if (std::min(m, n) / 2 < default_cfg().smin || !strassen_on() || !aligned || beta != 1.0 || (lower && m != n))
        return gemm_nt(m, n, k, alpha, A, lda, B, ldb, beta, C, ldc, lower, 0, st);
    std::vector<long long> plan;
    int rc = strassen_plan(m, n, k, lower, -1, -1, ~(size_t)0, plan);
    if (rc) return rc;
    const size_t need = plan_need(plan);
    if (!need) return run_plan(plan, alpha, A, lda, B, ldb, beta, C, ldc, nullptr, nullptr, st);
    const int dev = device_of(st);
    if (dev < 0) return gemm_nt(m, n, k, alpha, A, lda, B, ldb, beta, C, ldc, lower, 0, st);
    Scratch &s = g_scratch[dev];
    std::lock_guard<std::mutex> lock(s.mu);
    if (!scratch_ensure(s, need)) {
        if ((rc = strassen_plan(m, n, k, lower, -1, -1, s.cap, plan))) return rc;
        if (!plan_need(plan)) return run_plan(plan, alpha, A, lda, B, ldb, beta, C, ldc, nullptr, nullptr, st);
    }
    if (!s.ev) SGPR_HIP(hipEventCreateWithFlags(&s.ev, hipEventDisableTiming));
    if (s.used && s.last != st) SGPR_HIP(hipStreamWaitEvent(st, s.ev, 0));
    size_t na = 0;
    for (size_t i = 0; i + STRASSEN_REC <= plan.size(); i += STRASSEN_REC)
        if (plan[i] == PLAN_SUM && plan[i + 1] == 0) na = std::max(na, (size_t)plan[i + 2] * (size_t)plan[i + 3]);
    rc = run_plan(plan, alpha, A, lda, B, ldb, beta, C, ldc, s.p, s.p + na, st);
    SGPR_HIP(hipEventRecord(s.ev, st));
    s.last = st;
    s.used = true;
    return rc;
}

}
```

sympgpr_amd/csrc/gemm_tile.h:

```cpp
#pragma once
#include <type_traits>

#include "common.h"

namespace sgpr {
namespace tile {

typedef double double4_t __attribute__((ext_vector_type(4)));
typedef double double2_t __attribute__((ext_vector_type(2)));

#ifndef SGPR_GEMM_STAGES
#define SGPR_GEMM_STAGES 2
#endif
constexpr int BK = 16;
constexpr int PAD = 16;

struct GemmArgs {
    int m, n, k;
    double alpha, beta;
    const double *A;
    size_t lda;
    const double *B;
    size_t ldb;
    double *C;
    size_t ldc;
    int lower;
    long diag_off;
    int transb;
    unsigned long long *stamps;
    int tiles_m, tiles_n, n_sr, n_sc, n_super, tri;
    int n_full, n_grp;
    int lblk, lpr, lpi, lpc, lpj;
    int dbg;
    unsigned long long *kdone;
    double *C2;
    size_t ldc2;
    double alpha2;
};

constexpr int SR = 8;
template <int SC>
__device__ __forceinline__ bool tile_of(const GemmArgs &g, int &tile_r, int &tile_c)
{
    const int L = blockIdx.x;
    const int xcd = L & 7, j = L >> 3;
    const int S = (j / (SR * SC)) * 8 + xcd;
    if (S >= g.n_super) return false;
    const int w = j % (SR * SC);
    int sr, sc;
    if (!g.tri) {
        sc = S / g.n_sr;
        sr = S - sc * g.n_sr;
        if (g.lower) sr = (sr + sc) % g.n_sr;
    } else if (S < g.n_full) {
        const int N1 = g.n_sr - 1;
        const double nsr = (double)N1;
        int a = (int)((2.0 * nsr + 1.0 - sqrt((2.0 * nsr + 1.0) * (2.0 * nsr + 1.0) - 2.0 * (double)S)) * 0.5);
        if (a < 0) a = 0;
        while (a > 0 && 4 * (a * N1 - a * (a - 1) / 2) > S) --a;
        while (4 * ((a + 1) * N1 - (a + 1) * a / 2) <= S) ++a;
        const int rem = S - 4 * (a * N1 - a * (a - 1) / 2);
        const int per = N1 - a;
        const int b = rem / per;
        sc = 4 * a + b;
        sr = a + 1 + (rem - b * per);
    } else {
        const int d = S - g.n_full;
        const int b = d / g.n_grp, a = d - b * g.n_grp;
        sc = 4 * a + b;
        sr = a;
    }
    tile_r = sr * SR + (w % SR);
    tile_c = sc * SC + (w / SR);
    return tile_r < g.tiles_m && tile_c < g.tiles_n;
}

template <int BR, int THREADS, bool FAST>
__device__ __forceinline__ void load_tile(const double *P, size_t ld, int row0,
                                          int k0, int rows, int kmax, int tid,
                                          double2_t (&reg)[BR * BK / (2 * THREADS)])
{
    constexpr int PASSES = BR * BK / (2 * THREADS);
#pragma unroll
    for (int p = 0; p < PASSES; ++p) {
        const int e = p * THREADS + tid;
        const int r = 2 * (e % (BR / 2));
        const int kc = e / (BR / 2);
        if constexpr (FAST) {
            const double *src = P + (size_t)(row0 + r) + (size_t)(k0 + kc) * ld;
            reg[p] = *reinterpret_cast<const double2_t *>(src);
        } else {
            const int kk = min(k0 + kc, kmax - 1);
            const int r0 = min(row0 + r, rows - 1), r1 = min(row0 + r + 1, rows - 1);
            const double *col = P + (size_t)kk * ld;
            const double a = col[r0], b = col[r1];
            const bool kok = (k0 + kc) < kmax;
            double2_t v;
            v.x = (kok && (row0 + r) < rows) ? a : 0.0;
            v.y = (kok && (row0 + r + 1) < rows) ? b : 0.0;
            reg[p] = v;
        }
    }
}

template <int BR, int THREADS>
__device__ __forceinline__ void store_tile(double *S, int tid,
                                           const double2_t (&reg)[BR * BK / (2 * THREADS)])
{
    constexpr int PASSES = BR * BK / (2 * THREADS);
#pragma unroll
    for (int p = 0; p < PASSES; ++p) {
        const int e = p * THREADS + tid;
        const int r = 2 * (e % (BR / 2));
        const int kc = e / (BR / 2);
        *reinterpret_cast<double2_t *>(S + kc * (BR + PAD) + r) = reg[p];
    }
}

template <int BR, int THREADS, bool FAST>
__device__ __forceinline__ void load_tile_t(const double *P, size_t ld, int col0, int k0, int cols,
                                            int kmax, int tid, double2_t (&reg)[BR * BK / (2 * THREADS)])
{
    constexpr int PASSES = BR * BK / (2 * THREADS);
#pragma unroll
    for (int p = 0; p < PASSES; ++p) {
        const int e = p * THREADS + tid;
        const int kp = 2 * (e % (BK / 2));
        const int r = e / (BK / 2);
        if constexpr (FAST) {
            reg[p] = *reinterpret_cast<const double2_t *>(P + (size_t)(k0 + kp) + (size_t)(col0 + r) * ld);
        } else {
            const int cc = min(col0 + r, cols - 1);
            const int ka = min(k0 + kp, kmax - 1), kb = min(k0 + kp + 1, kmax - 1);
            const double *col = P + (size_t)cc * ld;
            const double a = col[ka], b = col[kb];
            const bool cok = (col0 + r) < cols;
            double2_t v;
            v.x = (cok && (k0 + kp) < kmax) ? a : 0.0;
            v.y = (cok && (k0 + kp + 1) < kmax) ? b : 0.0;
            reg[p] = v;
        }
    }
}
template <int BR, int THREADS>
__device__ __forceinline__ void store_pass_t(double *S, int tid, const double2_t &v, int p)
{
    const int e = p * THREADS + tid;
    const int kp = 2 * (e % (BK / 2));
    const int r = e / (BK / 2);
    S[kp * (BR + PAD) + r] = v.x;
    S[(kp + 1) * (BR + PAD) + r] = v.y;
}

template <int BR, int THREADS>
__device__ __forceinline__ void store_pass(double *S, int tid, const double2_t &v, int p)
{
    const int e = p * THREADS + tid;
    const int r = 2 * (e % (BR / 2));
    const int kc = e / (BR / 2);
    *reinterpret_cast<double2_t *>(S + kc * (BR + PAD) + r) = v;
}

template <int BM, int BN, bool FAST, bool TRANSB = false, bool TWO = false>
__device__ __forceinline__ void gemm_body(const GemmArgs &g, double *smem, int tile_r, int tile_c)
{
    constexpr int WGM = BM / 64, WGN = BN / 64;
    constexpr int THREADS = 64 * WGM * WGN;
    constexpr int LDA_S = BM + PAD, LDB_S = BN + PAD;
    constexpr int PA = BM * BK / (2 * THREADS), PB = BN * BK / (2 * THREADS);
    static_assert(PA >= 1 && PB >= 1, "tile too small for the thread count");
    double *const sA0 = smem;
    double *const sB0 = smem + 2 * BK * LDA_S;
    const int row0 = tile_r * BM;
    const int col0 = tile_c * BN;

    const int tid = threadIdx.x;
    const int lane = tid & 63;
    const int wave = tid >> 6;
    const int wm = wave % WGM, wn = wave / WGM;
    const int l15 = lane & 15, l4 = lane >> 4;


    double4_t acc[4][4];
#pragma unroll
    for (int i = 0; i < 4; ++i)
#pragma unroll
        for (int j = 0; j < 4; ++j) acc[i][j] = double4_t{0.0, 0.0, 0.0, 0.0};

    double2_t ra[PA], rb[PB];
    const int T = (g.k + BK - 1) / BK;
    unsigned long long st_c0 = 0, st_r0 = 0;
    if (g.stamps) { st_c0 = __builtin_amdgcn_s_memtime(); st_r0 = __builtin_amdgcn_s_memrealtime(); }

    auto fetch = [&](int t) {
        const int k0 = t * BK;
        load_tile<BM, THREADS, FAST>(g.A, g.lda, row0, k0, g.m, g.k, tid, ra);
        if constexpr (TRANSB) load_tile_t<BN, THREADS, FAST>(g.B, g.ldb, col0, k0, g.n, g.k, tid, rb);
        else                  load_tile<BN, THREADS, FAST>(g.B, g.ldb, col0, k0, g.n, g.k, tid, rb);
    };
    auto store_b = [&](double *S, int p) {
        if constexpr (TRANSB) store_pass_t<BN, THREADS>(S, tid, rb[p], p);
        else                  store_pass<BN, THREADS>(S, tid, rb[p], p);
    };

    double fa[2][4], fb[2][4];
    auto load_frags = [&](int buf, int kk, int set) {
        const double *sA = sA0 + buf * BK * LDA_S + wm * 64 + l15 + (kk * 4 + l4) * LDA_S;
        const double *sB = sB0 + buf * BK * LDB_S + wn * 64 + l15 + (kk * 4 + l4) * LDB_S;
#pragma unroll
        for (int i = 0; i < 4; ++i) {
            fa[set][i] = sB[i * 16];
            fb[set][i] = sA[i * 16];
        }
    };
    auto mfma_rows = [&](int set, int i0, int i1) {
#pragma unroll
        for (int i = i0; i < i1; ++i)
#pragma unroll
            for (int j = 0; j < 4; ++j)
                acc[i][j] = __builtin_amdgcn_mfma_f64_16x16x4f64(fa[set][i], fb[set][j], acc[i][j], 0, 0, 0);
    };

    if (T > 0) {
        fetch(0);
        store_tile<BM, THREADS>(sA0, tid, ra);
#pragma unroll
        for (int p = 0; p < PB; ++p) store_b(sB0, p);
        __syncthreads();
        load_frags(0, 0, 0);
    }
    for (int t = 0; t < T; ++t) {
        const int cur = t & 1;
        const bool more = t + 1 < T;
        if (more) fetch(t + 1);
        __builtin_amdgcn_sched_barrier(0);
        load_frags(cur, 1, 1);
        __builtin_amdgcn_sched_barrier(0);
        mfma_rows(0, 0, 4);
        __builtin_amdgcn_sched_barrier(0);
        load_frags(cur, 2, 0);
        __builtin_amdgcn_sched_barrier(0);
        mfma_rows(1, 0, 4);
        __builtin_amdgcn_sched_barrier(0);
        load_frags(cur, 3, 1);
        __builtin_amdgcn_sched_barrier(0);
        double *const nA = sA0 + (cur ^ 1) * BK * LDA_S;
        double *const nB = sB0 + (cur ^ 1) * BK * LDB_S;
#pragma unroll
        for (int i = 0; i < 4; ++i) {
            mfma_rows(0, i, i + 1);
            if (more) {
#pragma unroll
                for (int p = i * PA / 4; p < (i + 1) * PA / 4; ++p) store_pass<BM, THREADS>(nA, tid, ra[p], p);
#pragma unroll
                for (int p = i * PB / 4; p < (i + 1) * PB / 4; ++p) store_b(nB, p);
            }
            __builtin_amdgcn_sched_barrier(0);
        }
        mfma_rows(1, 0, 2);
        __builtin_amdgcn_sched_barrier(0);
        __syncthreads();
        if (more) load_frags(cur ^ 1, 0, 0);
        __builtin_amdgcn_sched_barrier(0);
        mfma_rows(1, 2, 4);
        __builtin_amdgcn_sched_barrier(0);
    }

    if (g.stamps && tid == 0) {
        unsigned long long *o = g.stamps + 4 * ((size_t)tile_c * g.tiles_m + tile_r);
        o[0] = st_c0; o[1] = __builtin_amdgcn_s_memtime();
        o[2] = st_r0; o[3] = __builtin_amdgcn_s_memrealtime();
    }

    const double alpha = g.alpha, beta = g.beta;
    const bool interior = (row0 + BM <= g.m) && (col0 + BN <= g.n);
#pragma unroll
    for (int i = 0; i < 4; ++i) {
        double old[4][4];
        if (beta != 0.0) {
#pragma unroll
            for (int r = 0; r < 4; ++r) {
                const int n = col0 + wn * 64 + i * 16 + 4 * r + l4;
#pragma unroll
                for (int j = 0; j < 4; ++j) {
                    const int m = row0 + wm * 64 + j * 16 + l15;
                    old[r][j] = (interior || (m < g.m && n < g.n)) ? g.C[(size_t)m + (size_t)n * g.ldc] : 0.0;
                }
            }
        }
        __builtin_amdgcn_sched_barrier(0);
#pragma unroll
        for (int r = 0; r < 4; ++r) {
            const int n = col0 + wn * 64 + i * 16 + 4 * r + l4;
#pragma unroll
            for (int j = 0; j < 4; ++j) {
                const int m = row0 + wm * 64 + j * 16 + l15;
                if (interior || (m < g.m && n < g.n)) {
                    const double v = alpha * acc[i][j][r];
                    g.C[(size_t)m + (size_t)n * g.ldc] = (beta == 0.0) ? v : __builtin_fma(beta, old[r][j], v);
                }
            }
        }
        __builtin_amdgcn_sched_barrier(0);
    }
    if constexpr (TWO) {
        const double alpha2 = g.alpha2;
#pragma unroll
        for (int i = 0; i < 4; ++i) {
            double old[4][4];
#pragma unroll
            for (int r = 0; r < 4; ++r) {
                const int n = col0 + wn * 64 + i * 16 + 4 * r + l4;
#pragma unroll
                for (int j = 0; j < 4; ++j) {
                    const int m = row0 + wm * 64 + j * 16 + l15;
                    old[r][j] = (interior || (m < g.m && n < g.n)) ? g.C2[(size_t)m + (size_t)n * g.ldc2] : 0.0;
                }
            }
            __builtin_amdgcn_sched_barrier(0);
#pragma unroll
            for (int r = 0; r < 4; ++r) {
                const int n = col0 + wn * 64 + i * 16 + 4 * r + l4;
#pragma unroll
                for (int j = 0; j < 4; ++j) {
                    const int m = row0 + wm * 64 + j * 16 + l15;
                    if (interior || (m < g.m && n < g.n))
                        g.C2[(size_t)m + (size_t)n * g.ldc2] = __builtin_fma(alpha2, acc[i][j][r], old[r][j]);
                }
            }
            __builtin_amdgcn_sched_barrier(0);
        }
    }
}

__device__ __forceinline__ unsigned lds_addr(const void *p)
{
    return (unsigned)(size_t)(const __attribute__((address_space(3))) void *)p;
}
template <int OFF>
__device__ __forceinline__ double ds_read_f64(unsigned addr)
{
    double v;
    asm volatile("ds_read_b64 %0, %1 offset:%2" : "=v"(v) : "v"(addr), "n"(OFF));
    return v;
}
template <int KK, int LDA_S, int LDB_S>
__device__ __forceinline__ void read_frags(unsigned aA, unsigned aB, double (&fa)[4], double (&fb)[4])
{
    fa[0] = ds_read_f64<(KK * 4 * LDB_S + 0) * 8>(aB);
    fb[0] = ds_read_f64<(KK * 4 * LDA_S + 0) * 8>(aA);
    fa[1] = ds_read_f64<(KK * 4 * LDB_S + 16) * 8>(aB);
    fb[1] = ds_read_f64<(KK * 4 * LDA_S + 16) * 8>(aA);
    fa[2] = ds_read_f64<(KK * 4 * LDB_S + 32) * 8>(aB);
    fb[2] = ds_read_f64<(KK * 4 * LDA_S + 32) * 8>(aA);
    fa[3] = ds_read_f64<(KK * 4 * LDB_S + 48) * 8>(aB);
    fb[3] = ds_read_f64<(KK * 4 * LDA_S + 48) * 8>(aA);
}
#define SGPR_LGKM_WAIT(n) do { asm volatile("s_waitcnt lgkmcnt(" #n ")" ::: "memory"); __builtin_amdgcn_sched_barrier(0); } while (0)

template <int BM, int BN, int STAGES, bool TWO = false>
__device__ __forceinline__ void gemm_body_dma(const GemmArgs &g, double *smem, int tile_r, int tile_c)
{
    constexpr int WGM = BM / 64, WGN = BN / 64;
    constexpr int NW = WGM * WGN;
    constexpr int LDA_S = BM + PAD, LDB_S = BN + PAD;
    constexpr int QA = BK * (BM / 128) / NW, QB = BK * (BN / 128) / NW;
    static_assert(QA >= 1 && QB >= 1 && BM % 128 == 0 && BN % 128 == 0, "tile / wave count mismatch");
    static_assert(STAGES == 2 || STAGES == 3, "two or three LDS stages");
    double *const sA0 = smem;
    double *const sB0 = smem + STAGES * BK * LDA_S;
    const int row0 = tile_r * BM, col0 = tile_c * BN;
    const int tid = threadIdx.x;
    const int lane = tid & 63;
    const int wave = __builtin_amdgcn_readfirstlane(tid >> 6);
    const int wm = wave % WGM, wn = wave / WGM;
    const int l15 = lane & 15, l4 = lane >> 4;

    double4_t acc[4][4];
#pragma unroll
    for (int i = 0; i < 4; ++i)
#pragma unroll
        for (int j = 0; j < 4; ++j) acc[i][j] = double4_t{0.0, 0.0, 0.0, 0.0};

    const int T = g.k / BK;
    unsigned long long st_c0 = 0, st_r0 = 0;
    if (g.stamps) { st_c0 = __builtin_amdgcn_s_memtime(); st_r0 = __builtin_amdgcn_s_memrealtime(); }

    const double *srcA[QA], *srcB[QB];
    int offA[QA], offB[QB];
#pragma unroll
    for (int j = 0; j < QA; ++j) {
        const int q = wave + NW * j, kc = q / (BM / 128), seg = q % (BM / 128);
        srcA[j] = g.A + (size_t)(row0 + seg * 128 + 2 * lane) + (size_t)kc * g.lda;
        offA[j] = kc * LDA_S + seg * 128;
    }
#pragma unroll
    for (int j = 0; j < QB; ++j) {
        const int q = wave + NW * j, kc = q / (BN / 128), seg = q % (BN / 128);
        srcB[j] = g.B + (size_t)(col0 + seg * 128 + 2 * lane) + (size_t)kc * g.ldb;
        offB[j] = kc * LDB_S + seg * 128;
    }
    const size_t stepA = (size_t)BK * g.lda, stepB = (size_t)BK * g.ldb;
    auto dma_one = [&](int t, int buf, int q) {
        if (q < QA) {
            __builtin_amdgcn_global_load_lds(
                (const __attribute__((address_space(1))) void *)(srcA[q] + (size_t)t * stepA),
                (__attribute__((address_space(3))) void *)(sA0 + buf * BK * LDA_S + offA[q]), 16, 0, 0);
        } else {
            __builtin_amdgcn_global_load_lds(
                (const __attribute__((address_space(1))) void *)(srcB[q - QA] + (size_t)t * stepB),
                (__attribute__((address_space(3))) void *)(sB0 + buf * BK * LDB_S + offB[q - QA]), 16, 0, 0);
        }
    };
    auto dma = [&](int t, int buf) {
#pragma unroll
        for (int q = 0; q < QA + QB; ++q) dma_one(t, buf, q);
    };
    constexpr int NQ = QA + QB;

    double fa0[4], fb0[4], fa1[4], fb1[4];
    auto mfma_rows = [&](const double (&fa)[4], const double (&fb)[4], int i0, int i1) {
#pragma unroll
        for (int i = i0; i < i1; ++i)
#pragma unroll
            for (int j = 0; j < 4; ++j)
                acc[i][j] = __builtin_amdgcn_mfma_f64_16x16x4f64(fa[i], fb[j], acc[i][j], 0, 0, 0);
    };
    const unsigned baseA = lds_addr(sA0 + wm * 64 + l15 + l4 * LDA_S);
    const unsigned baseB = lds_addr(sB0 + wn * 64 + l15 + l4 * LDB_S);

    constexpr int AHEAD = STAGES - 1;
    if (T > 0) {
        dma(0, 0);
        if (STAGES == 3 && T > 1) {
            dma(1, 1);
            asm volatile("s_waitcnt vmcnt(%0)" ::"n"(NQ) : "memory");
        } else {
            asm volatile("s_waitcnt vmcnt(0)" ::: "memory");
        }
        __builtin_amdgcn_s_barrier();
        read_frags<0, LDA_S, LDB_S>(baseA, baseB, fa0, fb0);
    }
    auto kstep = [&](int t, int cur, auto issue_tag, auto next_tag) {
        constexpr bool ISSUE = decltype(issue_tag)::value, NEXT = decltype(next_tag)::value;
        const int nxt = (cur + 1 == STAGES) ? 0 : cur + 1;
        const int tgt = (STAGES == 2) ? nxt : ((nxt + 1 == STAGES) ? 0 : nxt + 1);
        const unsigned aA = baseA + cur * (BK * LDA_S * 8), aB = baseB + cur * (BK * LDB_S * 8);
        __builtin_amdgcn_sched_barrier(0);
        read_frags<1, LDA_S, LDB_S>(aA, aB, fa1, fb1);
        SGPR_LGKM_WAIT(8);
#pragma unroll
        for (int i = 0; i < 4; ++i) {
            mfma_rows(fa0, fb0, i, i + 1);
            if constexpr (ISSUE) {
#pragma unroll
                for (int q = i * NQ / 8; q < (i + 1) * NQ / 8; ++q) dma_one(t + AHEAD, tgt, q);
            }
            __builtin_amdgcn_sched_barrier(0);
        }
        read_frags<2, LDA_S, LDB_S>(aA, aB, fa0, fb0);
        SGPR_LGKM_WAIT(8);
#pragma unroll
        for (int i = 0; i < 4; ++i) {
            mfma_rows(fa1, fb1, i, i + 1);
            if constexpr (ISSUE) {
#pragma unroll
                for (int q = (4 + i) * NQ / 8; q < (5 + i) * NQ / 8; ++q) dma_one(t + AHEAD, tgt, q);
            }
            __builtin_amdgcn_sched_barrier(0);
        }
        read_frags<3, LDA_S, LDB_S>(aA, aB, fa1, fb1);
        SGPR_LGKM_WAIT(8);
        mfma_rows(fa0, fb0, 0, 4);
        __builtin_amdgcn_sched_barrier(0);
        SGPR_LGKM_WAIT(0);
        mfma_rows(fa1, fb1, 0, 2);
        __builtin_amdgcn_sched_barrier(0);
        if constexpr (NEXT) {
            if constexpr (STAGES == 3 && ISSUE) asm volatile("s_waitcnt vmcnt(%0)" ::"n"(NQ) : "memory");
            else                                asm volatile("s_waitcnt vmcnt(0)" ::: "memory");
            __builtin_amdgcn_s_barrier();
            __builtin_amdgcn_sched_barrier(0);
            const unsigned nA = baseA + nxt * (BK * LDA_S * 8), nB = baseB + nxt * (BK * LDB_S * 8);
            read_frags<0, LDA_S, LDB_S>(nA, nB, fa0, fb0);
            __builtin_amdgcn_sched_barrier(0);
        }
        mfma_rows(fa1, fb1, 2, 4);
        __builtin_amdgcn_sched_barrier(0);
        return nxt;
    };
    {
        int t = 0, cur = 0;
        for (; t + AHEAD < T; ++t) cur = kstep(t, cur, std::true_type(), std::true_type());
        for (; t + 1 < T; ++t) cur = kstep(t, cur, std::false_type(), std::true_type());
        if (t < T) kstep(t, cur, std::false_type(), std::false_type());
    }
    SGPR_LGKM_WAIT(0);

    if (g.stamps && tid == 0) {
        unsigned long long *o = g.stamps + 4 * ((size_t)tile_c * g.tiles_m + tile_r);
        o[0] = st_c0; o[1] = __builtin_amdgcn_s_memtime();
        o[2] = st_r0; o[3] = __builtin_amdgcn_s_memrealtime();
    }
    if (g.kdone && tid == 0) *g.kdone = __builtin_amdgcn_s_memrealtime();

    const double alpha = g.alpha, beta = g.beta;
    double *const cbase = g.C + (size_t)(row0 + wm * 64 + l15) + (size_t)(col0 + wn * 64 + l4) * g.ldc;
    double old[2][4][4];
    auto fetch = [&](int i, double (&o)[4][4]) {
#pragma unroll
        for (int r = 0; r < 4; ++r)
#pragma unroll
            for (int j = 0; j < 4; ++j) o[r][j] = cbase[(size_t)(j * 16) + (size_t)(i * 16 + 4 * r) * g.ldc];
    };
    if (beta != 0.0) fetch(0, old[0]);
#pragma unroll
    for (int i = 0; i < 4; ++i) {
        if (beta != 0.0 && i + 1 < 4) fetch(i + 1, old[(i + 1) & 1]);
        __builtin_amdgcn_sched_barrier(0);
        if (beta != 0.0) {
            if (i + 1 < 4) asm volatile("s_waitcnt vmcnt(16)" ::: "memory");
            else           asm volatile("s_waitcnt vmcnt(0)" ::: "memory");
        }
        __builtin_amdgcn_sched_barrier(0);
#pragma unroll
        for (int r = 0; r < 4; ++r)
#pragma unroll
            for (int j = 0; j < 4; ++j) {
                const double v = alpha * acc[i][j][r];
                cbase[(size_t)(j * 16) + (size_t)(i * 16 + 4 * r) * g.ldc] = (beta == 0.0) ? v : __builtin_fma(beta, old[i & 1][r][j], v);
            }
        __builtin_amdgcn_sched_barrier(0);
    }
    if constexpr (TWO) {
        const double alpha2 = g.alpha2;
        double *const cbase2 = g.C2 + (size_t)(row0 + wm * 64 + l15) + (size_t)(col0 + wn * 64 + l4) * g.ldc2;
        auto fetch2 = [&](int i, double (&o)[4][4]) {
#pragma unroll
            for (int r = 0; r < 4; ++r)
#pragma unroll
                for (int j = 0; j < 4; ++j) o[r][j] = cbase2[(size_t)(j * 16) + (size_t)(i * 16 + 4 * r) * g.ldc2];
        };
        fetch2(0, old[0]);
#pragma unroll
        for (int i = 0; i < 4; ++i) {
            if (i + 1 < 4) fetch2(i + 1, old[(i + 1) & 1]);
            __builtin_amdgcn_sched_barrier(0);
            if (i + 1 < 4) asm volatile("s_waitcnt vmcnt(16)" ::: "memory");
            else           asm volatile("s_waitcnt vmcnt(0)" ::: "memory");
            __builtin_amdgcn_sched_barrier(0);
#pragma unroll
            for (int r = 0; r < 4; ++r)
#pragma unroll
                for (int j = 0; j < 4; ++j)
                    cbase2[(size_t)(j * 16) + (size_t)(i * 16 + 4 * r) * g.ldc2] = __builtin_fma(alpha2, acc[i][j][r], old[i & 1][r][j]);
            __builtin_amdgcn_sched_barrier(0);
        }
    }
}


}
}
```

sympgpr_amd/csrc/probe.hip:

```cpp
#include <algorithm>
#include <cstdlib>
#include <vector>

#include "cholq.h"
#include "common.h"
#include "../../include/sympgpr_probe.h"
#include "generated/pair_generated.h"

namespace sgpr {
namespace {
typedef double double4_t __attribute__((ext_vector_type(4)));
typedef double double2_t __attribute__((ext_vector_type(2)));

template <int NACC>
__global__ __launch_bounds__(256) void mfma_clock_kernel(int iters, double *out, unsigned long long *stamps)
{
    double4_t acc[NACC];
    const double a = 1.0 + threadIdx.x * 1e-9, b = 1.0 - threadIdx.x * 1e-9;
#pragma unroll
    for (int i = 0; i < NACC; ++i) acc[i] = double4_t{0.0, 0.0, 0.0, 0.0};
    const unsigned long long t0 = __builtin_amdgcn_s_memtime(), r0 = __builtin_amdgcn_s_memrealtime();
    for (int it = 0; it < iters; ++it) {
#pragma unroll
        for (int i = 0; i < NACC; ++i)
// ... 197 lines not shown
#pragma unroll
    for (int r = 0; r < 4; ++r) { D[r] = (4 * r + l4 == l15) ? 4.0 + 0.01 * l15 : 1.0 / (2.0 + l15 + 4 * r + l4); X[r] = (4 * r + l4 == l15) ? 1.0 : 0.0; }
    double rl = io[0], acc = io[1];
    auto bcast = [&](double v, int ln) {
        const unsigned lo = __builtin_amdgcn_readlane((int)__double2loint(v), ln);
        const unsigned hi = __builtin_amdgcn_readlane((int)__double2hiint(v), ln);
        return __hiloint2double((int)hi, (int)lo);
    };
    auto nr = [&](double d) {
        double r = __builtin_amdgcn_rsq(d);
        r = r * __builtin_fma(-0.5 * d * r, r, 1.5);
        r = r * __builtin_fma(-0.5 * d * r, r, 1.5);
        return r;
    };
    unsigned long long t0, t1;
    asm volatile("s_memtime %0\n\ts_waitcnt lgkmcnt(0)" : "=s"(t0), "+v"(rl), "+v"(acc), "+v"(D), "+v"(X) : : "memory");
#pragma unroll
    for (int j = 0; j < 16; ++j) {
        const int rj = j >> 2;
        if (V == 0) {
            const double v = D[rj] * rl;
            D = __builtin_amdgcn_mfma_f64_16x16x4f64(v, v, D, 0, 0, 0);
        } else if (V == 1) {
            const double v = D[rj] * rl, x = X[rj] * rl;
            D = __builtin_amdgcn_mfma_f64_16x16x4f64(v, v, D, 0, 0, 0);
            X = __builtin_amdgcn_mfma_f64_16x16x4f64(v, x, X, 0, 0, 0);
        } else if (V == 2) {
            const double a = bcast(acc, (j + 1) & 63), b = bcast(rl, (j + 17) & 63);
            rl = nr(__builtin_fma(-b, b, a + 5.0));
            acc += rl;
        } else if (V == 3) {
            rl = __builtin_amdgcn_rsq(rl + 1.0);
        } else if (V == 4) {
#pragma unroll
            for (int q = 0; q < 8; ++q) rl = __builtin_fma(rl, acc, 0.5);
        } else if (V == 5) {
            rl = bcast(rl, (j + 1) & 63) + acc;
        } else if (V == 6) {
            sh[lane] = rl;
            rl = sh[(lane + 1) & 63] + 1.0;
        } else if (V >= 8) {
            const int g = j & 3;
            const double v = D[rj] * rl;
            const double x = X[rj] * rl;
            double rn = 0.0;
            if (j + 1 < 16) {
                const double dnext = bcast(D[(j + 1) >> 2], (j + 1) + 16 * ((j + 1) & 3));
                const double lnext = bcast(v, (j + 1) + 16 * g);
                rn = nr(__builtin_fma(-lnext, lnext, dnext));
            }
            if (V == 8 || V == 9) {
                if (l4 == g) big[j * 130 + l15] = v;
                sh[j] = rl;
            }
            const double nv = v * mneg[j];
            D = __builtin_amdgcn_mfma_f64_16x16x4f64(nv, v, D, 0, 0, 0);
            if (V == 8 || V == 10) X = __builtin_amdgcn_mfma_f64_16x16x4f64(nv, x, X, 0, 0, 0);
            rl = rn;
        } else if (V == 7) {
            const double v = D[rj] * rl;
            D = __builtin_amdgcn_mfma_f64_16x16x4f64(v, v, D, 0, 0, 0);
            rl = bcast(D[0], 0) * 1e-3;
        }
    }
    double ssum = rl + acc + D[0] + D[1] + D[2] + D[3] + X[0] + X[1] + X[2] + X[3];
    asm volatile("s_nop 0\n\ts_memtime %0\n\ts_waitcnt lgkmcnt(0)" : "=s"(t1), "+v"(ssum) : : "memory");
    if (lane == 0) cyc[V] = t1 - t0;
    if (ssum == 12345.678) io[2] = ssum + big[lane] + sh[lane];
}
} }

extern "C" int sgpr_probe_lat(double *out8 )
{
    double *io = nullptr;
    unsigned long long *cyc = nullptr;
    SGPR_HIP(hipMalloc((void **)&io, 64));
    SGPR_HIP(hipMalloc((void **)&cyc, 128));
    const double h[3] = {0.49, 1.25, 0.0};
    SGPR_HIP(hipMemcpy(io, h, sizeof(h), hipMemcpyHostToDevice));
    for (int rep = 0; rep < 2; ++rep) {
        hipLaunchKernelGGL((sgpr::lat_probe_kernel<0>), dim3(1), dim3(256), 0, 0, io, cyc);
        hipLaunchKernelGGL((sgpr::lat_probe_kernel<1>), dim3(1), dim3(256), 0, 0, io, cyc);
        hipLaunchKernelGGL((sgpr::lat_probe_kernel<2>), dim3(1), dim3(256), 0, 0, io, cyc);
        hipLaunchKernelGGL((sgpr::lat_probe_kernel<3>), dim3(1), dim3(256), 0, 0, io, cyc);
        hipLaunchKernelGGL((sgpr::lat_probe_kernel<4>), dim3(1), dim3(256), 0, 0, io, cyc);
        hipLaunchKernelGGL((sgpr::lat_probe_kernel<5>), dim3(1), dim3(256), 0, 0, io, cyc);
        hipLaunchKernelGGL((sgpr::lat_probe_kernel<6>), dim3(1), dim3(256), 0, 0, io, cyc);
        hipLaunchKernelGGL((sgpr::lat_probe_kernel<7>), dim3(1), dim3(256), 0, 0, io, cyc);
        hipLaunchKernelGGL((sgpr::lat_probe_kernel<8>), dim3(1), dim3(256), 0, 0, io, cyc);
        hipLaunchKernelGGL((sgpr::lat_probe_kernel<9>), dim3(1), dim3(256), 0, 0, io, cyc);
        hipLaunchKernelGGL((sgpr::lat_probe_kernel<10>), dim3(1), dim3(256), 0, 0, io, cyc);
        hipLaunchKernelGGL((sgpr::lat_probe_kernel<11>), dim3(1), dim3(256), 0, 0, io, cyc);
        SGPR_HIP(hipDeviceSynchronize());
    }
    unsigned long long hs[12];
    SGPR_HIP(hipMemcpy(hs, cyc, 96, hipMemcpyDeviceToHost));
    for (int i = 0; i < 12; ++i) out8[i] = (double)hs[i] / 16.0;
    (void)hipFree(io); (void)hipFree(cyc);
    return 0;
}

extern "C" int sgpr_probe_leaf(double *out8)
{
    const int n = LEAF;
    std::vector<double> h((size_t)n * n, 0.0);
    for (int i = 0; i < n; ++i)
        for (int j = 0; j <= i; ++j) h[i + (size_t)j * n] = (i == j) ? 4.0 + 0.01 * i : 1.0 / (1.0 + i + j);
    double *A = nullptr, *inv = nullptr;
    int *info = nullptr;
    unsigned long long *st = nullptr;
    SGPR_HIP(hipMalloc((void **)&A, sizeof(double) * n * n));
    SGPR_HIP(hipMalloc((void **)&inv, sizeof(double) * n * n));
    SGPR_HIP(hipMalloc((void **)&info, 16));
    SGPR_HIP(hipMalloc((void **)&st, 64));
    SGPR_HIP(hipMemset(info, 0, 16));
    for (int rep = 0; rep < 2; ++rep) {
        SGPR_HIP(hipMemcpy(A, h.data(), sizeof(double) * n * n, hipMemcpyHostToDevice));
        int rc = leaf_probe(A, n, inv, info, st, nullptr);
        if (rc) return rc;
        SGPR_HIP(hipDeviceSynchronize());
    }
    unsigned long long hs[8];
    SGPR_HIP(hipMemcpy(hs, st, 64, hipMemcpyDeviceToHost));
    for (int i = 0; i < 8; ++i) out8[i] = (double)hs[i];
    (void)hipFree(A); (void)hipFree(inv); (void)hipFree(info); (void)hipFree(st);
    return 0;
}

namespace sgpr { namespace {
__global__ __launch_bounds__(512) void xcc_probe_kernel(int *out)
{
    const int x = __builtin_amdgcn_s_getreg(20 | (0 << 6) | (3 << 11));
    if (threadIdx.x == 0) out[blockIdx.x] = x;
    unsigned long long t0 = __builtin_amdgcn_s_memtime();
    while (__builtin_amdgcn_s_memtime() - t0 < 20000) {}
}
} }
extern "C" int sgpr_probe_xcc(int nblocks, int *host_out)
{
    int *d = nullptr;
    SGPR_HIP(hipMalloc((void **)&d, sizeof(int) * nblocks));
    hipLaunchKernelGGL(sgpr::xcc_probe_kernel, dim3(nblocks), dim3(512), 0, nullptr, d);
    SGPR_HIP(hipMemcpy(host_out, d, sizeof(int) * nblocks, hipMemcpyDeviceToHost));
    (void)hipFree(d);
    return 0;
}

namespace sgpr { namespace {
__global__ __launch_bounds__(512) void cumask_probe_kernel(int *out)
{
    const int x = __builtin_amdgcn_s_getreg(20 | (0 << 6) | (3 << 11));
    const int hw = __builtin_amdgcn_s_getreg(4 | (0 << 6) | (31 << 11));
    if (threadIdx.x == 0) { out[2 * blockIdx.x] = x; out[2 * blockIdx.x + 1] = hw; }
    unsigned long long t0 = __builtin_amdgcn_s_memtime();
    while (__builtin_amdgcn_s_memtime() - t0 < 200000) {}
}
} }
extern "C" int sgpr_probe_cumask(const unsigned *mask_words, int nwords, int nblocks, int *host_out)
{
    hipStream_t st = nullptr;
    SGPR_HIP(hipExtStreamCreateWithCUMask(&st, (uint32_t)nwords, mask_words));
    int *d = nullptr;
    SGPR_HIP(hipMalloc((void **)&d, sizeof(int) * 2 * nblocks));
    hipLaunchKernelGGL(sgpr::cumask_probe_kernel, dim3(nblocks), dim3(512), 0, st, d);
    SGPR_HIP(hipStreamSynchronize(st));
    SGPR_HIP(hipMemcpy(host_out, d, sizeof(int) * 2 * nblocks, hipMemcpyDeviceToHost));
    (void)hipFree(d);
    (void)hipStreamDestroy(st);
    return 0;
}


namespace sgpr {
template <int FAM>
__global__ void generated_eval_kernel(int which, int m, const double *xa, const double *ya, const double *xb,
                                      const double *yb, double lx, double ly, double p, double *out)
{
    const int i = blockIdx.x * blockDim.x + threadIdx.x;
    if (i >= m) return;
    double o[4];
    const int dl = which >> 2;
    if (dl == 0)      gen::pair<FAM>(xa[i], ya[i], xb[i], yb[i], lx, ly, p, o);
    else if (dl == 1) gen::pair_dlx<FAM>(xa[i], ya[i], xb[i], yb[i], lx, ly, p, o);
    else              gen::pair_dly<FAM>(xa[i], ya[i], xb[i], yb[i], lx, ly, p, o);
    out[i] = o[which & 3];
}
}

extern "C" int sgpr_probe_generated_eval(int family, int which, int m, const double *xa, const double *ya,
                                         const double *xb, const double *yb, const double *l, int nl, double *out)
{
    using namespace sgpr;
    if (m <= 0) return 0;
    if (which < 0 || which > 11 || !l || nl < 2 || (family == SGPR_FAM_D && nl < 3)) { set_error("generated_eval: bad arguments"); return SGPR_E_ARG; }
    double *d[5] = {};
    const double *h[4] = {xa, ya, xb, yb};
    for (int k = 0; k < 5; ++k) SGPR_HIP(hipMalloc((void **)&d[k], sizeof(double) * m));
    for (int k = 0; k < 4; ++k) SGPR_HIP(hipMemcpy(d[k], h[k], sizeof(double) * m, hipMemcpyHostToDevice));
    const double p = family == SGPR_FAM_D ? l[2] : 0.0;
    const dim3 grid((m + 255) / 256);
    switch (family) {
    case SGPR_FAM_A: hipLaunchKernelGGL(generated_eval_kernel<SGPR_FAM_A>, grid, dim3(256), 0, nullptr, which, m, d[0], d[1], d[2], d[3], l[0], l[1], p, d[4]); break;
    case SGPR_FAM_B: hipLaunchKernelGGL(generated_eval_kernel<SGPR_FAM_B>, grid, dim3(256), 0, nullptr, which, m, d[0], d[1], d[2], d[3], l[0], l[1], p, d[4]); break;
    case SGPR_FAM_C: hipLaunchKernelGGL(generated_eval_kernel<SGPR_FAM_C>, grid, dim3(256), 0, nullptr, which, m, d[0], d[1], d[2], d[3], l[0], l[1], p, d[4]); break;
    case SGPR_FAM_D: hipLaunchKernelGGL(generated_eval_kernel<SGPR_FAM_D>, grid, dim3(256), 0, nullptr, which, m, d[0], d[1], d[2], d[3], l[0], l[1], p, d[4]); break;
    default: set_error("unknown kernel family"); return SGPR_E_ARG;
    }
    SGPR_CHECK_LAUNCH();
    SGPR_HIP(hipMemcpy(out, d[4], sizeof(double) * m, hipMemcpyDeviceToHost));
    for (int k = 0; k < 5; ++k) (void)hipFree(d[k]);
    return 0;
}

extern "C" int sgpr_probe_queue_plan(int n, int nworkers, int *starts_out, int max_starts, unsigned *tasks_out,
                                     int max_tasks, int *counts)
{
    cholq::Plan p;
    const int rc = cholq::build_plan(n, cholq::default_starts(n), nworkers, p);
    if (rc) return rc;
    counts[0] = p.nblk;
    counts[1] = (int)(p.tasks.size() / 2);
    counts[2] = (int)p.model_us;
    for (int k = 0; k <= p.nblk && k < max_starts; ++k) starts_out[k] = p.starts[k];
    for (size_t t = 0; t < p.tasks.size() && (int)(t / 2) < max_tasks; ++t) tasks_out[t] = p.tasks[t];
    return 0;
}

extern "C" int sgpr_probe_queue_plan_partial(int n, int nworkers, int nq, int *starts_out, int max_starts, unsigned *tasks_out,
                                             int max_tasks, int *counts)
{
    cholq::Plan p;
    const std::vector<int> st = cholq::default_starts(n);
    const int rc = cholq::build_plan(n, st, nworkers, p, nq < 0 ? cholq::default_nq(n, st) : nq);
    if (rc) return rc;
    counts[0] = p.nblk;
    counts[1] = (int)(p.tasks.size() / 2);
    counts[2] = (int)p.model_us;
    counts[3] = p.nq;
    for (int k = 0; k <= p.nblk && k < max_starts; ++k) starts_out[k] = p.starts[k];
    for (size_t t = 0; t < p.tasks.size() && (int)(t / 2) < max_tasks; ++t) tasks_out[t] = p.tasks[t];
    return 0;
}

static unsigned long long *g_qtrace = nullptr;
static int g_qtrace_cap = 0;
extern "C" int sgpr_probe_queue_trace_begin(int max_tasks)
{
    if (g_qtrace) { cholq::set_trace(nullptr, 0); (void)hipFree(g_qtrace); g_qtrace = nullptr; }
    SGPR_HIP(hipMalloc((void **)&g_qtrace, sizeof(unsigned long long) * cholq::trace_words((size_t)max_tasks)));
    SGPR_HIP(hipMemset(g_qtrace, 0, sizeof(unsigned long long) * cholq::trace_words((size_t)max_tasks)));
    g_qtrace_cap = max_tasks;
    cholq::set_trace(g_qtrace, (size_t)max_tasks);
    return max_tasks;
}
extern "C" int sgpr_probe_queue_trace_clear()
{
    if (!g_qtrace) return 0;
    SGPR_HIP(hipMemset(g_qtrace, 0, sizeof(unsigned long long) * cholq::trace_words((size_t)g_qtrace_cap)));
    return 0;
}
extern "C" int sgpr_probe_queue_trace_end(unsigned long long *out, int max_tasks)
{
    if (!g_qtrace) return 0;
    SGPR_HIP(hipDeviceSynchronize());
    cholq::set_trace(nullptr, 0);
    if (max_tasks < g_qtrace_cap) { set_error("queue_trace_end: buffer smaller than the capacity given to _begin"); return SGPR_E_ARG; }
    const size_t words = cholq::trace_words((size_t)g_qtrace_cap);
    SGPR_HIP(hipMemcpy(out, g_qtrace, sizeof(unsigned long long) * words, hipMemcpyDeviceToHost));
    (void)hipFree(g_qtrace);
    g_qtrace = nullptr;
    return (int)words;
}

extern "C" int sgpr_probe_queue_postmortem(int always) { return cholq::postmortem(always != 0); }
extern "C" int sgpr_probe_queue_force_giveup(int on) { cholq::force_giveup(on); return 0; }
extern "C" int sgpr_probe_tune(const char *name, double value)
{
    if (!name) { set_error("probe_tune: null name"); return SGPR_E_ARG; }
    tune_set(name, value);
    return 0;
}

extern "C" int sgpr_probe_strassen_plan(int m, int n, int k, int lower, long smin, long kslab, long scratch_doubles, long long *out,
                                        int max_records, int *count)
{
    if (!count || scratch_doubles < 0) { set_error("probe_strassen_plan: bad arguments"); return SGPR_E_ARG; }
    std::vector<long long> plan;
    const int rc = strassen_plan(m, n, k, lower, smin, kslab, (size_t)scratch_doubles, plan);
    if (rc) return rc;
    *count = (int)(plan.size() / STRASSEN_REC);
    for (size_t i = 0; out && i < plan.size() && (int)(i / STRASSEN_REC) < max_records; ++i) out[i] = plan[i];
    return 0;
}
extern "C" int sgpr_probe_gemm_strassen_dev(int m, int n, int k, double alpha, const double *A, size_t lda, const double *B, size_t ldb,
                                            double beta, double *C, size_t ldc, int lower, void *stream)
{
    return gemm_nt_strassen(m, n, k, alpha, A, lda, B, ldb, beta, C, ldc, lower, static_cast<hipStream_t>(stream));
}
extern "C" int sgpr_probe_gemm_nt2_dev(int m, int n, int k, double alpha, const double *A, size_t lda, const double *B, size_t ldb,
                                       double beta, double *C, size_t ldc, double alpha2, double *C2, size_t ldc2, void *stream)
{
    return gemm_nt_two(m, n, k, alpha, A, lda, B, ldb, beta, C, ldc, alpha2, C2, ldc2, static_cast<hipStream_t>(stream));
}
extern "C" unsigned sgpr_probe_map_calls(void) { return applymap_last_calls(); }
extern "C" int sgpr_probe_map_team(int ntest, int n0) { return applymap_team(ntest, n0); }
extern "C" int sgpr_probe_trsm_piece(int ticket, int cap, int strips, int out[5]) { if (ticket < 0 || cap < 1 || strips < 0 || !out) return SGPR_E_ARG; trsm_piece_of(ticket, cap, strips, out); return 0; }
extern "C" int sgpr_probe_trsm_counts(int strips, int cap, unsigned long long out[2])
{
    if (strips < 0 || cap < 1 || !out) return SGPR_E_ARG;
    size_t c[2];
    trsm_piece_counts(strips, cap, c);
    out[0] = c[0]; out[1] = c[1];
    return 0;
}

namespace sgpr { namespace {
__global__ void census_kernel(unsigned long long *out, int spin_us)
{
    extern __shared__ double dyn[];
    const unsigned long long t0 = __builtin_amdgcn_s_memrealtime();
    if (threadIdx.x == 0) {
        dyn[0] = 1.0;
        out[4 * blockIdx.x + 0] = (unsigned long long)__builtin_amdgcn_s_getreg(20 | (0 << 6) | (3 << 11));
        out[4 * blockIdx.x + 1] = (unsigned long long)__builtin_amdgcn_s_getreg(4 | (0 << 6) | (31 << 11));
        out[4 * blockIdx.x + 2] = t0;
    }
    while (__builtin_amdgcn_s_memrealtime() - t0 < (unsigned long long)spin_us * 100ull) __builtin_amdgcn_s_sleep(32);
    if (threadIdx.x == 0) out[4 * blockIdx.x + 3] = __builtin_amdgcn_s_memrealtime();
}
} }
extern "C" int sgpr_probe_census(int na, int threads_a, int lds_a, int spin_a, const unsigned *mask_a, int nwords_a,
                                 int nb, int threads_b, int lds_b, int spin_b, const unsigned *mask_b, int nwords_b,
                                 unsigned long long *host_out)
{
    hipStream_t sa = nullptr, sb = nullptr;
    if (nwords_a > 0) SGPR_HIP(hipExtStreamCreateWithCUMask(&sa, (uint32_t)nwords_a, mask_a));
    else              SGPR_HIP(hipStreamCreateWithFlags(&sa, hipStreamNonBlocking));
    if (nwords_b > 0) SGPR_HIP(hipExtStreamCreateWithCUMask(&sb, (uint32_t)nwords_b, mask_b));
    else {
        int lo = 0, hi = 0;
        SGPR_HIP(hipDeviceGetStreamPriorityRange(&lo, &hi));
        SGPR_HIP(hipStreamCreateWithPriority(&sb, hipStreamNonBlocking, hi));
    }
    unsigned long long *d = nullptr;
    const size_t words = 4 * (size_t)(na + nb);
    SGPR_HIP(hipMalloc((void **)&d, sizeof(unsigned long long) * words));
    SGPR_HIP(hipMemset(d, 0, sizeof(unsigned long long) * words));
    SGPR_HIP(hipFuncSetAttribute((const void *)sgpr::census_kernel, hipFuncAttributeMaxDynamicSharedMemorySize, 160 * 1024));
    SGPR_HIP(hipDeviceSynchronize());
    hipLaunchKernelGGL(sgpr::census_kernel, dim3(na), dim3(threads_a), lds_a, sa, d, spin_a);
    SGPR_CHECK_LAUNCH();
    hipLaunchKernelGGL(sgpr::census_kernel, dim3(nb), dim3(threads_b), lds_b, sb, d + 4 * (size_t)na, spin_b);
    SGPR_CHECK_LAUNCH();
    SGPR_HIP(hipStreamSynchronize(sa));
    SGPR_HIP(hipStreamSynchronize(sb));
    SGPR_HIP(hipMemcpy(host_out, d, sizeof(unsigned long long) * words, hipMemcpyDeviceToHost));
    (void)hipFree(d);
    (void)hipStreamDestroy(sa);
    (void)hipStreamDestroy(sb);
    return 0;
}
```

Baseline: 76.32.

## Add two-level Strassen for large fp64 GEMM updates with multi-destination epilogue

```diff
diff --git a/include/sympgpr_probe.h b/include/sympgpr_probe.h
--- a/include/sympgpr_probe.h
+++ b/include/sympgpr_probe.h
@@ -34,6 +34,10 @@
                                  double beta, double *C, size_t ldc, int lower, void *stream);
 int sgpr_probe_gemm_nt2_dev(int m, int n, int k, double alpha, const double *A, size_t lda, const double *B, size_t ldb,
                             double beta, double *C, size_t ldc, double alpha2, double *C2, size_t ldc2, void *stream);
+int sgpr_probe_strassen2_plan(int m, int n, int k, int lower, long smin, long kslab, long smin2, long kslab2, long scratch_doubles,
+                              long long *out, int max_records, int *count);
+int sgpr_probe_gemm_nt4_dev(int m, int n, int k, const double *A, size_t lda, const double *B, size_t ldb, double beta, int count,
+                            double *const *C, const size_t *ldc, const double *alpha, void *stream);
 unsigned sgpr_probe_map_calls(void);
 int sgpr_probe_map_team(int ntest, int n0);
 
diff --git a/sympgpr_amd/_lib.py b/sympgpr_amd/_lib.py
--- a/sympgpr_amd/_lib.py
+++ b/sympgpr_amd/_lib.py
@@ -156,6 +156,10 @@
                                                C.c_double, C.c_void_p, C.c_size_t, C.c_int, C.c_void_p]),
     "sgpr_probe_gemm_nt2_dev": (C.c_int, [C.c_int, C.c_int, C.c_int, C.c_double, C.c_void_p, C.c_size_t, C.c_void_p, C.c_size_t,
                                           C.c_double, C.c_void_p, C.c_size_t, C.c_double, C.c_void_p, C.c_size_t, C.c_void_p]),
+    "sgpr_probe_strassen2_plan": (C.c_int, [C.c_int, C.c_int, C.c_int, C.c_int, C.c_long, C.c_long, C.c_long, C.c_long, C.c_long,
+                                            C.POINTER(C.c_longlong), C.c_int, C.POINTER(C.c_int)]),
+    "sgpr_probe_gemm_nt4_dev": (C.c_int, [C.c_int, C.c_int, C.c_int, C.c_void_p, C.c_size_t, C.c_void_p, C.c_size_t, C.c_double, C.c_int,
+                                          C.POINTER(C.c_void_p), C.POINTER(C.c_size_t), C.POINTER(C.c_double), C.c_void_p]),
     "sgpr_probe_census": (C.c_int, [C.c_int, C.c_int, C.c_int, C.c_int, C.POINTER(C.c_uint), C.c_int,
                                     C.c_int, C.c_int, C.c_int, C.c_int, C.POINTER(C.c_uint), C.c_int,
                                     C.POINTER(C.c_ulonglong)]),
diff --git a/sympgpr_amd/csrc/chol.hip b/sympgpr_amd/csrc/chol.hip
--- a/sympgpr_amd/csrc/chol.hip
+++ b/sympgpr_amd/csrc/chol.hip
@@ -1464,7 +1464,10 @@
     c.strassen = true;
     if (n > c.la_max && n > LEAF) {
         const int n1 = split(n), n2 = n - n1, n11 = split(n1);
-        strassen_reserve(std::max(strassen_scratch_doubles(n2, n2, n1, 1), strassen_scratch_doubles(n2, n1 - n11, n11, 0)), st);
+        auto need = [&](int levels) {
+            return std::max(strassen_scratch_doubles(n2, n2, n1, 1, levels), strassen_scratch_doubles(n2, n1 - n11, n11, 0, levels));
+        };
+        strassen_reserve(need(2), need(1), st);
     }
     const bool dbg = PANEL_DBG && getenv("SGPR_PANEL_DBG") != nullptr;
     const int T = (n + LEAF - 1) / LEAF;
diff --git a/sympgpr_amd/csrc/common.h b/sympgpr_amd/csrc/common.h
--- a/sympgpr_amd/csrc/common.h
+++ b/sympgpr_amd/csrc/common.h
@@ -86,8 +86,13 @@
 int gemm_nt_strassen(int m, int n, int k, double alpha, const double *A, size_t lda, const double *B, size_t ldb, double beta,
                      double *C, size_t ldc, int lower, hipStream_t st);
 int strassen_plan(int m, int n, int k, int lower, long smin, long kslab, size_t scratch_doubles, std::vector<long long> &out);
-size_t strassen_scratch_doubles(int m, int n, int k, int lower);
-void strassen_reserve(size_t doubles, hipStream_t st);
+enum { PLAN2_SUM = 4, PLAN2_PROD = 5 };
+int strassen_outer_plan(int m, int n, int k, int lower, long smin, long kslab, long smin2, long kslab2, size_t scratch_doubles,
+                   std::vector<long long> &out);
+int gemm_nt_multi(int m, int n, int k, const double *A, size_t lda, const double *B, size_t ldb, double beta, int count,
+                  double *const *C, const size_t *ldc, const double *alpha, hipStream_t st);
+size_t strassen_scratch_doubles(int m, int n, int k, int lower, int levels);
+void strassen_reserve(size_t both, size_t one, hipStream_t st);
 int strassen_trim();
 int gemm_profile_begin();
 int gemm_profile_end(double *out12);
diff --git a/sympgpr_amd/csrc/gemm_f64.hip b/sympgpr_amd/csrc/gemm_f64.hip
--- a/sympgpr_amd/csrc/gemm_f64.hip
+++ b/sympgpr_amd/csrc/gemm_f64.hip
@@ -65,6 +65,21 @@
     if (fast) gemm_body_dma<BM, BN, SGPR_GEMM_STAGES, true>(g, smem, tile_r, tile_c);
     else      gemm_body<BM, BN, false, false, true>(g, smem, tile_r, tile_c);
 }
+
+__global__ __launch_bounds__(512, 2) void gemm_nt4_kernel(const GemmArgs g)
+{
+    constexpr int BM = 256, BN = 128, LDA_S = BM + PAD, LDB_S = BN + PAD;
+    __shared__ double smem[SGPR_GEMM_STAGES * BK * (LDA_S + LDB_S)];
+    int tile_r, tile_c;
+    if (!tile_of<(SR * BM) / (4 * BN)>(g, tile_r, tile_c)) return;
+    const int row0 = tile_r * BM, col0 = tile_c * BN;
+    const bool aligned = ((((uintptr_t)g.A | (uintptr_t)g.B) & 15) == 0) && (((g.lda | g.ldb) & 1) == 0);
+    const bool fast = aligned && (row0 + BM <= g.m) && (col0 + BN <= g.n) && (g.k % BK == 0);
+    if (fast) gemm_body_dma<BM, BN, SGPR_GEMM_STAGES, false, true>(g, smem, tile_r, tile_c);
+    else      gemm_body<BM, BN, false, false, false, true>(g, smem, tile_r, tile_c);
+}
+
+struct Dst { double *C; size_t ld; double alpha; };
 
 __global__ __launch_bounds__(256) void block_sum_kernel(int rows, int cols, const double *X, size_t ldx, const double *Y, size_t ldy,
                                                         double sign, double *T)
@@ -102,12 +117,12 @@
 
 static int gemm_launch(int m, int n, int k, double alpha, const double *A, size_t lda, const double *B,
                        size_t ldb, double beta, double *C, size_t ldc, int lower, const int *bc, int transb,
-                       hipStream_t st, unsigned long long *stamps = nullptr, int dbg = 0, double *C2 = nullptr,
-                       size_t ldc2 = 0, double alpha2 = 0.0);
+                       hipStream_t st, unsigned long long *stamps = nullptr, int dbg = 0, const Dst *x = nullptr, int nx = 0,
+                       bool k4 = false);
 
 static int gemm_chunked(int m, int n, int k, double alpha, const double *A, size_t lda, const double *B,
                         size_t ldb, double beta, double *C, size_t ldc, int lower, const int *bc,
-                        hipStream_t st, double *C2, size_t ldc2, double alpha2)
+                        hipStream_t st, const Dst *x, int nx, bool k4)
 {
     static const int kmax = [] { const char *e = getenv("SGPR_GEMM_KMAX"); return e ? atoi(e) : 8192; }();
     if (kmax >= 128 && k > kmax) {
@@ -115,19 +130,19 @@
         const int step = ((k + nchunk - 1) / nchunk + 127) / 128 * 128;
         for (int k0 = 0; k0 < k; k0 += step) {
             const int rc = gemm_launch(m, n, std::min(step, k - k0), alpha, A + (size_t)k0 * lda, lda, B + (size_t)k0 * ldb, ldb,
-                                       k0 == 0 ? beta : 1.0, C, ldc, lower, bc, 0, st, nullptr, 0, C2, ldc2, alpha2);
+                                       k0 == 0 ? beta : 1.0, C, ldc, lower, bc, 0, st, nullptr, 0, x, nx, k4);
             if (rc) return rc;
         }
         return 0;
     }
-    return gemm_launch(m, n, k, alpha, A, lda, B, ldb, beta, C, ldc, lower, bc, 0, st, nullptr, 0, C2, ldc2, alpha2);
+    return gemm_launch(m, n, k, alpha, A, lda, B, ldb, beta, C, ldc, lower, bc, 0, st, nullptr, 0, x, nx, k4);
 }
 
 int gemm_nt_bc(int m, int n, int k, double alpha, const double *A, size_t lda, const double *B,
                size_t ldb, double beta, double *C, size_t ldc, int lower, const int *bc,
                hipStream_t st)
 {
-    return gemm_chunked(m, n, k, alpha, A, lda, B, ldb, beta, C, ldc, lower, bc, st, nullptr, 0, 0.0);
+    return gemm_chunked(m, n, k, alpha, A, lda, B, ldb, beta, C, ldc, lower, bc, st, nullptr, 0, false);
 }
 
 int gemm_nt_two(int m, int n, int k, double alpha, const double *A, size_t lda, const double *B, size_t ldb, double beta,
@@ -135,12 +150,26 @@
 {
     const int bc[5] = {1, 1, 0, 1, 0};
     if (!C2) { set_error("gemm_nt_two: null second destination"); return SGPR_E_ARG; }
-    return gemm_chunked(m, n, k, alpha, A, lda, B, ldb, beta, C, ldc, 0, bc, st, C2, ldc2, alpha2);
+    const Dst x{C2, ldc2, alpha2};
+    return gemm_chunked(m, n, k, alpha, A, lda, B, ldb, beta, C, ldc, 0, bc, st, &x, 1, false);
+}
+
+int gemm_nt_multi(int m, int n, int k, const double *A, size_t lda, const double *B, size_t ldb, double beta, int count,
+                  double *const *C, const size_t *ldc, const double *alpha, hipStream_t st)
+{
+    const int bc[5] = {1, 1, 0, 1, 0};
+    if (count < 2 || count > 4 || !C || !ldc || !alpha) { set_error("gemm_nt_multi: 2 to 4 destinations"); return SGPR_E_ARG; }
+    Dst x[3];
+    for (int d = 0; d < count; ++d) {
+        if (!C[d]) { set_error("gemm_nt_multi: null destination"); return SGPR_E_ARG; }
+        if (d) x[d - 1] = Dst{C[d], ldc[d], alpha[d]};
+    }
+    return gemm_chunked(m, n, k, alpha[0], A, lda, B, ldb, beta, C[0], ldc[0], 0, bc, st, x, count - 1, true);
 }
 
 static int gemm_launch(int m, int n, int k, double alpha, const double *A, size_t lda, const double *B,
                        size_t ldb, double beta, double *C, size_t ldc, int lower, const int *bc, int transb,
-                       hipStream_t st, unsigned long long *stamps, int dbg, double *C2, size_t ldc2, double alpha2)
+                       hipStream_t st, unsigned long long *stamps, int dbg, const Dst *x, int nx, bool k4)
 {
     const bool plain = bc[0] == 1 && bc[1] == 1 && bc[3] == 1 && bc[4] == 0;
     const long diag_off = plain ? bc[2] : 1;
@@ -151,9 +180,15 @@
         set_error("gemm: leading dimension too small");
         return SGPR_E_ARG;
     }
-    if (C2 && (lower || transb || ldc2 < (size_t)m)) { set_error("gemm: bad second destination"); return SGPR_E_ARG; }
+    if (nx < 0 || nx > 3 || (nx && !x)) { set_error("gemm: bad destination count"); return SGPR_E_ARG; }
+    Dst d[3] = {};
+    for (int i = 0; i < nx; ++i) {
+        d[i] = x[i];
+        if (!d[i].C || lower || transb || d[i].ld < (size_t)m) { set_error("gemm: bad second destination"); return SGPR_E_ARG; }
+    }
     GemmArgs g{m, n, k, alpha, beta, A, lda, B, ldb, C, ldc, lower, diag_off, transb, stamps, 0, 0, 0, 0, 0, 0,
-               0, 0, bc[0], bc[1], bc[2], bc[3], bc[4], dbg, nullptr, C2, ldc2, alpha2};
+               0, 0, bc[0], bc[1], bc[2], bc[3], bc[4], dbg, nullptr, d[0].C, d[0].ld, d[0].alpha,
+               d[1].C, d[1].ld, d[1].alpha, d[2].C, d[2].ld, d[2].alpha, nx + 1};
     auto set_map = [&](int bm, int bn) {
         g.tiles_m = (m + bm - 1) / bm;
         g.tiles_n = (n + bn - 1) / bn;
@@ -212,9 +247,10 @@
     static const double small_mb = tune("gemm_small_mb", 0.0);
     const double op_bytes = 8.0 * (double)k * ((A == B && lda == ldb) ? (double)std::max(m, n) : (double)m + n);
     const bool small_k = op_bytes <= small_mb * 1e6 && m > 128 && n > 128;
-    if (C2) {
+    if (nx) {
         const dim3 grid(set_map(256, 128));
-        hipLaunchKernelGGL(gemm_nt2_kernel, grid, dim3(512), 0, st, g);
+        if (k4 || nx > 1) hipLaunchKernelGGL(gemm_nt4_kernel, grid, dim3(512), 0, st, g);
+        else              hipLaunchKernelGGL(gemm_nt2_kernel, grid, dim3(512), 0, st, g);
         rec.big = 1;
     } else if (n <= 128 && m <= 32768 && !(dbg & 8)) {
         const dim3 grid(set_map(64, 128));
@@ -338,38 +374,39 @@
     if (!step) return false;
     return (size_t)(m / 2 + n / 2) * (size_t)(step / 2) <= c.scratch;
 }
+void seven(int kind_sum, int kind_prod, long m2, long n2, long k2, long k0, long ar, long br, long cr, long cc, std::vector<long long> &out)
+{
+    const long a1 = ar, a2 = ar + m2, b1 = br, b2 = br + n2, j1 = k0, j2 = k0 + k2;
+    const long c1r = cr, c2r = cr + m2, c1c = cc, c2c = cc + n2;
+    auto sum = [&](int side, long xr, long xc, long yr, long yc, int sign) {
+        put(out, {kind_sum, side, side ? n2 : m2, k2, xr, xc, yr, yc, sign});
+    };
+    auto prod = [&](int as, long pr, long pc, int bs, long qr, long qc, long d1r, long d1c, int s1, long d2r, long d2c, int s2) {
+        put(out, {kind_prod, as, pr, pc, bs, qr, qc, m2, n2, k2, d1r, d1c, s1, d2r, d2c, s2});
+    };
+    sum(0, a1, j1, a2, j2, +1); sum(1, b1, j1, b2, j2, +1);
+    prod(1, 0, 0, 1, 0, 0, c1r, c1c, +1, c2r, c2c, +1);
+    sum(0, a2, j1, a2, j2, +1);
+    prod(1, 0, 0, 0, b1, j1, c2r, c1c, +1, c2r, c2c, -1);
+    sum(1, b2, j1, b2, j2, -1);
+    prod(0, a1, j1, 1, 0, 0, c1r, c2c, +1, c2r, c2c, +1);
+    sum(1, b1, j2, b1, j1, -1);
+    prod(0, a2, j2, 1, 0, 0, c1r, c1c, +1, c2r, c1c, +1);
+    sum(0, a1, j1, a1, j2, +1);
+    prod(1, 0, 0, 0, b2, j2, c1r, c1c, -1, c1r, c2c, +1);
+    sum(0, a2, j1, a1, j1, -1); sum(1, b1, j1, b2, j1, +1);
+    prod(1, 0, 0, 1, 0, 0, c2r, c2c, +1, 0, 0, 0);
+    sum(0, a1, j2, a2, j2, -1); sum(1, b1, j2, b2, j2, +1);
+    prod(1, 0, 0, 1, 0, 0, c1r, c1c, +1, 0, 0, 0);
+}
 void plan_gemm(long m, long n, long k, long ar, long br, long cr, long cc, const PlanCfg &c, std::vector<long long> &out)
 {
     if (!qualifies(m, n, k, c)) {
         put(out, {PLAN_CLASSIC, 0, ar, 0, br, 0, m, n, k, cr, cc});
         return;
     }
-    const long m2 = m / 2, n2 = n / 2, step = slab_of(k, c);
-    for (long k0 = 0; k0 < k; k0 += step) {
-        const long k2 = std::min(step, k - k0) / 2;
-        const long a1 = ar, a2 = ar + m2, b1 = br, b2 = br + n2, j1 = k0, j2 = k0 + k2;
-        const long c1r = cr, c2r = cr + m2, c1c = cc, c2c = cc + n2;
-        auto sum = [&](int side, long xr, long xc, long yr, long yc, int sign) {
-            put(out, {PLAN_SUM, side, side ? n2 : m2, k2, xr, xc, yr, yc, sign});
-        };
-        auto prod = [&](int as, long pr, long pc, int bs, long qr, long qc, long d1r, long d1c, int s1, long d2r, long d2c, int s2) {
-            put(out, {PLAN_PROD, as, pr, pc, bs, qr, qc, m2, n2, k2, d1r, d1c, s1, d2r, d2c, s2});
-        };
-        sum(0, a1, j1, a2, j2, +1); sum(1, b1, j1, b2, j2, +1);
-        prod(1, 0, 0, 1, 0, 0, c1r, c1c, +1, c2r, c2c, +1);
-        sum(0, a2, j1, a2, j2, +1);
-        prod(1, 0, 0, 0, b1, j1, c2r, c1c, +1, c2r, c2c, -1);
-        sum(1, b2, j1, b2, j2, -1);
-        prod(0, a1, j1, 1, 0, 0, c1r, c2c, +1, c2r, c2c, +1);
-        sum(1, b1, j2, b1, j1, -1);
-        prod(0, a2, j2, 1, 0, 0, c1r, c1c, +1, c2r, c1c, +1);
-        sum(0, a1, j1, a1, j2, +1);
-        prod(1, 0, 0, 0, b2, j2, c1r, c1c, -1, c1r, c2c, +1);
-        sum(0, a2, j1, a1, j1, -1); sum(1, b1, j1, b2, j1, +1);
-        prod(1, 0, 0, 1, 0, 0, c2r, c2c, +1, 0, 0, 0);
-        sum(0, a1, j2, a2, j2, -1); sum(1, b1, j2, b2, j2, +1);
-        prod(1, 0, 0, 1, 0, 0, c1r, c1c, +1, 0, 0, 0);
-    }
+    const long step = slab_of(k, c);
+    for (long k0 = 0; k0 < k; k0 += step) seven(PLAN_SUM, PLAN_PROD, m / 2, n / 2, std::min(step, k - k0) / 2, k0, ar, br, cr, cc, out);
 }
 void plan_syrk(long n, long k, long r0, const PlanCfg &c, std::vector<long long> &out)
 {
@@ -390,16 +427,103 @@
     return need[0] + need[1];
 }
 
-bool strassen_on()
-{
-    static const bool on = [] { const char *e = getenv("SGPR_GEMM_STRASSEN"); return !(e && e[0] == '0'); }();
-    return on;
-}
+int strassen_levels()
+{
+    static const int lv = [] { const char *e = getenv("SGPR_GEMM_STRASSEN"); return !e ? 2 : (e[0] == '0' ? 0 : (e[0] == '1' ? 1 : 2)); }();
+    return lv;
+}
+bool strassen_on() { return strassen_levels() > 0; }
 PlanCfg default_cfg()
 {
     static const long smin = std::max(128L, (long)tune("gemm_strassen_min", 8192));
     static const long kslab = std::max(32L, (long)tune("gemm_strassen_kslab", 16384));
     return PlanCfg{smin, kslab, ~(size_t)0};
+}
+
+struct Plan2Cfg {
+    PlanCfg in;
+    long smin2;
+    long kslab2;
+    size_t scratch;
+};
+Plan2Cfg default_cfg2()
+{
+    static const long smin2 = std::max(256L, (long)tune("gemm_strassen2_min", 16384));
+    static const long kslab2 = std::max(64L, (long)tune("gemm_strassen2_kslab", 32768));
+    return Plan2Cfg{default_cfg(), smin2, kslab2, ~(size_t)0};
+}
+bool outer_noscratch()
+{
+    static const bool forced_fail = tune("gemm_strassen2_noscratch", 0) != 0;
+    return forced_fail;
+}
+bool qualifies2(long m, long n, long k, const Plan2Cfg &c)
+{
+    if (m <= 0 || n <= 0 || m % 1024 != 0 || n % 512 != 0) return false;
+    if (m / 2 < c.smin2 || n / 2 < c.smin2) return false;
+    if (c.kslab2 < 64 || c.kslab2 % 64 != 0 || k < c.kslab2) return false;
+    const size_t pair = (size_t)(m / 2 + n / 2) * (size_t)(c.kslab2 / 2);
+    if (pair > c.scratch) return false;
+    PlanCfg ci = c.in;
+    ci.scratch = c.scratch - pair;
+    return qualifies(m / 2, n / 2, c.kslab2 / 2, ci);
+}
+PlanCfg inner_of(const Plan2Cfg &c)
+{
+    PlanCfg ci = c.in;
+    ci.scratch = c.scratch;
+    return ci;
+}
+void plan2_gemm(long m, long n, long k, long ar, long br, long cr, long cc, const Plan2Cfg &c, std::vector<long long> &out)
+{
+    if (!qualifies2(m, n, k, c)) { plan_gemm(m, n, k, ar, br, cr, cc, inner_of(c), out); return; }
+    long k0 = 0;
+    for (; k0 + c.kslab2 <= k; k0 += c.kslab2) seven(PLAN2_SUM, PLAN2_PROD, m / 2, n / 2, c.kslab2 / 2, k0, ar, br, cr, cc, out);
+    if (k0 == k) return;
+    size_t i = out.size();
+    plan_gemm(m, n, k - k0, ar, br, cr, cc, inner_of(c), out);
+    for (; i + STRASSEN_REC <= out.size(); i += STRASSEN_REC) {
+        long long *r = &out[i];
+        if (r[0] == PLAN_SUM) { r[5] += k0; r[7] += k0; }
+        else if (r[0] == PLAN_PROD) { if (!r[1]) r[3] += k0; if (!r[4]) r[6] += k0; }
+        else { r[3] += k0; r[5] += k0; }
+    }
+}
+void plan2_syrk(long n, long k, long r0, const Plan2Cfg &c, std::vector<long long> &out)
+{
+    const long h = n / 2;
+    if (n % 2 != 0 || !qualifies2(h, h, k, c)) { plan_syrk(n, k, r0, inner_of(c), out); return; }
+    plan2_syrk(h, k, r0, c, out);
+    plan2_gemm(h, h, k, r0 + h, r0, r0 + h, r0, c, out);
+    plan2_syrk(h, k, r0 + h, c, out);
+}
+void inner_plan(const long long *r, const PlanCfg &ci, std::vector<long long> &out)
+{
+    out.clear();
+    plan_gemm(r[7], r[8], r[9], 0, 0, 0, 0, ci, out);
+}
+struct Need2 { size_t v[4] = {0, 0, 0, 0}; size_t inner() const { return v[0] + v[1]; } size_t total() const { return v[0] + v[1] + v[2] + v[3]; } };
+Need2 plan2_need(const std::vector<long long> &plan, const Plan2Cfg &c)
+{
+    Need2 nd;
+    std::vector<long long> in;
+    auto sums = [&](const long long *r, int base) {
+        size_t &v = nd.v[base + r[1]];
+        v = std::max(v, (size_t)r[2] * (size_t)r[3]);
+    };
+    PlanCfg ci = c.in;
+    ci.scratch = ~(size_t)0;
+    for (size_t i = 0; i + STRASSEN_REC <= plan.size(); i += STRASSEN_REC) {
+        const long long *r = &plan[i];
+        if (r[0] == PLAN_SUM) sums(r, 0);
+        else if (r[0] == PLAN2_SUM) sums(r, 2);
+        else if (r[0] == PLAN2_PROD) {
+            inner_plan(r, ci, in);
+            for (size_t j = 0; j + STRASSEN_REC <= in.size(); j += STRASSEN_REC)
+                if (in[j] == PLAN_SUM) sums(&in[j], 0);
+        }
+    }
+    return nd;
 }
 
 struct Scratch {
@@ -443,11 +567,11 @@
     return 0;
 }
 
-int run_plan(const std::vector<long long> &plan, double alpha, const double *A, size_t lda, const double *B, size_t ldb,
-             double beta, double *C, size_t ldc, double *SA, double *SB, hipStream_t st)
-{
-    for (size_t i = 0; i + STRASSEN_REC <= plan.size(); i += STRASSEN_REC) {
-        const long long *r = &plan[i];
+int run_plan(const long long *recs, size_t nrec, double alpha, const double *A, size_t lda, const double *B, size_t ldb,
+             double beta, double *C, size_t ldc, double alpha2, double *C2, size_t ldc2, double *SA, double *SB, hipStream_t st)
+{
+    for (size_t i = 0; i < nrec; ++i) {
+        const long long *r = recs + i * STRASSEN_REC;
         int rc = 0;
         if (r[0] == PLAN_SUM) {
             const double *P = r[1] ? B : A;
@@ -458,13 +582,67 @@
             const int m = (int)r[7], n = (int)r[8], k = (int)r[9];
             const double *Ap = r[1] ? SA : A + r[2] + (size_t)r[3] * lda;
             const double *Bp = r[4] ? SB : B + r[5] + (size_t)r[6] * ldb;
+            const size_t la = r[1] ? (size_t)m : lda, lb = r[4] ? (size_t)n : ldb;
             double *C1 = C + r[10] + (size_t)r[11] * ldc;
-            if (r[15]) rc = gemm_nt_two(m, n, k, alpha * (double)r[12], Ap, r[1] ? (size_t)m : lda, Bp, r[4] ? (size_t)n : ldb, 1.0, C1, ldc,
-                                     alpha * (double)r[15], C + r[13] + (size_t)r[14] * ldc, ldc, st);
-            else       rc = gemm_nt(m, n, k, alpha * (double)r[12], Ap, r[1] ? (size_t)m : lda, Bp, r[4] ? (size_t)n : ldb, 1.0, C1, ldc, 0, 0, st);
+            if (C2) {
+                double *cs[4] = {C1, nullptr, nullptr, nullptr};
+                size_t ls[4] = {ldc, 0, 0, 0};
+                double as[4] = {alpha * (double)r[12], 0.0, 0.0, 0.0};
+                int cnt = 1;
+                auto add = [&](double *p, size_t l, double a) { cs[cnt] = p; ls[cnt] = l; as[cnt] = a; ++cnt; };
+                if (r[15]) add(C + r[13] + (size_t)r[14] * ldc, ldc, alpha * (double)r[15]);
+                add(C2 + r[10] + (size_t)r[11] * ldc2, ldc2, alpha2 * (double)r[12]);
+                if (r[15]) add(C2 + r[13] + (size_t)r[14] * ldc2, ldc2, alpha2 * (double)r[15]);
+                if (cnt == 2) rc = gemm_nt_two(m, n, k, as[0], Ap, la, Bp, lb, 1.0, cs[0], ls[0], as[1], cs[1], ls[1], st);
+                else          rc = gemm_nt_multi(m, n, k, Ap, la, Bp, lb, 1.0, cnt, cs, ls, as, st);
+            } else if (r[15]) {
+                rc = gemm_nt_two(m, n, k, alpha * (double)r[12], Ap, la, Bp, lb, 1.0, C1, ldc,
+                                 alpha * (double)r[15], C + r[13] + (size_t)r[14] * ldc, ldc, st);
+            } else {
+                rc = gemm_nt(m, n, k, alpha * (double)r[12], Ap, la, Bp, lb, 1.0, C1, ldc, 0, 0, st);
+            }
+        } else if (r[0] == PLAN_CLASSIC) {
+            const double *Ap = A + r[2] + (size_t)r[3] * lda, *Bp = B + r[4] + (size_t)r[5] * ldb;
+            if (C2) rc = gemm_nt_two((int)r[6], (int)r[7], (int)r[8], alpha, Ap, lda, Bp, ldb, beta, C + r[9] + (size_t)r[10] * ldc, ldc,
+                                     alpha2, C2 + r[9] + (size_t)r[10] * ldc2, ldc2, st);
+            else    rc = gemm_nt((int)r[6], (int)r[7], (int)r[8], alpha, Ap, lda, Bp, ldb, beta, C + r[9] + (size_t)r[10] * ldc, ldc, (int)r[1], 0, st);
         } else {
-            rc = gemm_nt((int)r[6], (int)r[7], (int)r[8], alpha, A + r[2] + (size_t)r[3] * lda, lda, B + r[4] + (size_t)r[5] * ldb, ldb,
-                         beta, C + r[9] + (size_t)r[10] * ldc, ldc, (int)r[1], 0, st);
+            set_error("run_plan: unknown record");
+            rc = SGPR_E_ARG;
+        }
+        if (rc) return rc;
+    }
+    return 0;
+}
+int run_plan(const std::vector<long long> &plan, double alpha, const double *A, size_t lda, const double *B, size_t ldb,
+             double beta, double *C, size_t ldc, double *SA, double *SB, hipStream_t st)
+{
+    return run_plan(plan.data(), plan.size() / STRASSEN_REC, alpha, A, lda, B, ldb, beta, C, ldc, 0.0, nullptr, 0, SA, SB, st);
+}
+int run_plan2(const std::vector<long long> &plan, const Plan2Cfg &c, const Need2 &nd, double alpha, const double *A, size_t lda,
+              const double *B, size_t ldb, double beta, double *C, size_t ldc, double *S, hipStream_t st)
+{
+    double *const SA = S, *const SB = S + nd.v[0], *const OA = SB + nd.v[1], *const OB = OA + nd.v[2];
+    PlanCfg ci = c.in;
+    ci.scratch = nd.inner();
+    std::vector<long long> in;
+    for (size_t i = 0; i + STRASSEN_REC <= plan.size(); i += STRASSEN_REC) {
+        const long long *r = &plan[i];
+        int rc = 0;
+        if (r[0] == PLAN2_SUM) {
+            const double *P = r[1] ? B : A;
+            const size_t ld = r[1] ? ldb : lda;
+            rc = block_sum((int)r[2], (int)r[3], P + r[4] + (size_t)r[5] * ld, ld, P + r[6] + (size_t)r[7] * ld, ld, (double)r[8],
+                           r[1] ? OB : OA, st);
+        } else if (r[0] == PLAN2_PROD) {
+            const double *X = r[1] ? OA : A + r[2] + (size_t)r[3] * lda;
+            const double *Y = r[4] ? OB : B + r[5] + (size_t)r[6] * ldb;
+            inner_plan(r, ci, in);
+            rc = run_plan(in.data(), in.size() / STRASSEN_REC, alpha * (double)r[12], X, r[1] ? (size_t)r[7] : lda, Y, r[4] ? (size_t)r[8] : ldb,
+                          1.0, C + r[10] + (size_t)r[11] * ldc, ldc, alpha * (double)r[15], r[15] ? C + r[13] + (size_t)r[14] * ldc : nullptr, ldc,
+                          SA, SB, st);
+        } else {
+            rc = run_plan(r, 1, alpha, A, lda, B, ldb, beta, C, ldc, 0.0, nullptr, 0, SA, SB, st);
         }
         if (rc) return rc;
     }
@@ -485,20 +663,50 @@
     return 0;
 }
 
-size_t strassen_scratch_doubles(int m, int n, int k, int lower)
+namespace {
+Plan2Cfg cfg2_of(long smin, long kslab, long smin2, long kslab2, size_t scratch_doubles)
+{
+    Plan2Cfg c = default_cfg2();
+    if (smin >= 0) c.in.smin = std::max(128L, smin);
+    if (kslab >= 0) c.in.kslab = std::max(32L, kslab);
+    if (smin2 >= 0) c.smin2 = std::max(256L, smin2);
+    if (kslab2 >= 0) c.kslab2 = std::max(64L, kslab2);
+    c.scratch = scratch_doubles;
+    return c;
+}
+}
+
+int strassen_outer_plan(int m, int n, int k, int lower, long smin, long kslab, long smin2, long kslab2, size_t scratch_doubles,
+                   std::vector<long long> &out)
+{
+    if (m < 0 || n < 0 || k < 0 || (lower && m != n)) { set_error("strassen_outer_plan: bad extents"); return SGPR_E_ARG; }
+    const Plan2Cfg c = cfg2_of(smin, kslab, smin2, kslab2, scratch_doubles);
+    out.clear();
+    if (lower) plan2_syrk(n, k, 0, c, out);
+    else       plan2_gemm(m, n, k, 0, 0, 0, 0, c, out);
+    return 0;
+}
+
+size_t strassen_scratch_doubles(int m, int n, int k, int lower, int levels)
 {
     std::vector<long long> plan;
-    if (!strassen_on() || strassen_plan(m, n, k, lower, -1, -1, ~(size_t)0, plan)) return 0;
+    if (!strassen_on()) return 0;
+    if (levels >= 2 && strassen_levels() >= 2) {
+        if (strassen_outer_plan(m, n, k, lower, -1, -1, -1, -1, ~(size_t)0, plan)) return 0;
+        return plan2_need(plan, default_cfg2()).total();
+    }
+    if (strassen_plan(m, n, k, lower, -1, -1, ~(size_t)0, plan)) return 0;
     return plan_need(plan);
 }
 
-void strassen_reserve(size_t doubles, hipStream_t st)
+void strassen_reserve(size_t both, size_t one, hipStream_t st)
 {
     const int dev = device_of(st);
-    if (!doubles || dev < 0 || !strassen_on()) return;
+    if (dev < 0 || !strassen_on()) return;
     Scratch &s = g_scratch[dev];
     std::lock_guard<std::mutex> lock(s.mu);
-    (void)scratch_ensure(s, doubles);
+    if (both > one && !outer_noscratch() && scratch_ensure(s, both)) return;
+    if (one) (void)scratch_ensure(s, one);
 }
 
 int strassen_trim()
@@ -520,11 +728,32 @@
     if (std::min(m, n) / 2 < default_cfg().smin || !strassen_on() || !aligned || beta != 1.0 || (lower && m != n))
         return gemm_nt(m, n, k, alpha, A, lda, B, ldb, beta, C, ldc, lower, 0, st);
     std::vector<long long> plan;
-    int rc = strassen_plan(m, n, k, lower, -1, -1, ~(size_t)0, plan);
+    int rc = 0;
+    const int dev = device_of(st);
+    auto enqueue = [&](Scratch &s, auto &&run) {
+        if (!s.ev) SGPR_HIP(hipEventCreateWithFlags(&s.ev, hipEventDisableTiming));
+        if (s.used && s.last != st) SGPR_HIP(hipStreamWaitEvent(st, s.ev, 0));
+        const int r = run();
+        SGPR_HIP(hipEventRecord(s.ev, st));
+        s.last = st;
+        s.used = true;
+        return r;
+    };
+    const Plan2Cfg c2 = default_cfg2();
+    if (strassen_levels() >= 2 && dev >= 0 && !outer_noscratch() && std::min(lower ? m / 2 : m, lower ? n / 2 : n) / 2 >= c2.smin2) {
+        if ((rc = strassen_outer_plan(m, n, k, lower, -1, -1, -1, -1, ~(size_t)0, plan))) return rc;
+        const Need2 nd = plan2_need(plan, c2);
+        if (nd.v[2] + nd.v[3]) {
+            Scratch &s = g_scratch[dev];
+            std::lock_guard<std::mutex> lock(s.mu);
+            if (scratch_ensure(s, nd.total()))
+                return enqueue(s, [&] { return run_plan2(plan, c2, nd, alpha, A, lda, B, ldb, beta, C, ldc, s.p, st); });
+        }
+    }
+    rc = strassen_plan(m, n, k, lower, -1, -1, ~(size_t)0, plan);
     if (rc) return rc;
     const size_t need = plan_need(plan);
     if (!need) return run_plan(plan, alpha, A, lda, B, ldb, beta, C, ldc, nullptr, nullptr, st);
-    const int dev = device_of(st);
     if (dev < 0) return gemm_nt(m, n, k, alpha, A, lda, B, ldb, beta, C, ldc, lower, 0, st);
     Scratch &s = g_scratch[dev];
     std::lock_guard<std::mutex> lock(s.mu);
@@ -532,16 +761,10 @@
         if ((rc = strassen_plan(m, n, k, lower, -1, -1, s.cap, plan))) return rc;
         if (!plan_need(plan)) return run_plan(plan, alpha, A, lda, B, ldb, beta, C, ldc, nullptr, nullptr, st);
     }
-    if (!s.ev) SGPR_HIP(hipEventCreateWithFlags(&s.ev, hipEventDisableTiming));
-    if (s.used && s.last != st) SGPR_HIP(hipStreamWaitEvent(st, s.ev, 0));
     size_t na = 0;
     for (size_t i = 0; i + STRASSEN_REC <= plan.size(); i += STRASSEN_REC)
         if (plan[i] == PLAN_SUM && plan[i + 1] == 0) na = std::max(na, (size_t)plan[i + 2] * (size_t)plan[i + 3]);
-    rc = run_plan(plan, alpha, A, lda, B, ldb, beta, C, ldc, s.p, s.p + na, st);
-    SGPR_HIP(hipEventRecord(s.ev, st));
-    s.last = st;
-    s.used = true;
-    return rc;
-}
-
-}
+    return enqueue(s, [&] { return run_plan(plan, alpha, A, lda, B, ldb, beta, C, ldc, s.p, s.p + na, st); });
+}
+
+}
diff --git a/sympgpr_amd/csrc/gemm_tile.h b/sympgpr_amd/csrc/gemm_tile.h
--- a/sympgpr_amd/csrc/gemm_tile.h
+++ b/sympgpr_amd/csrc/gemm_tile.h
@@ -36,6 +36,13 @@
     double *C2;
     size_t ldc2;
     double alpha2;
+    double *C3;
+    size_t ldc3;
+    double alpha3;
+    double *C4;
+    size_t ldc4;
+    double alpha4;
+    int ndst;
 };
 
 constexpr int SR = 8;
@@ -161,7 +168,7 @@
     *reinterpret_cast<double2_t *>(S + kc * (BR + PAD) + r) = v;
 }
 
-template <int BM, int BN, bool FAST, bool TRANSB = false, bool TWO = false>
+template <int BM, int BN, bool FAST, bool TRANSB = false, bool TWO = false, bool FOUR = false>
 __device__ __forceinline__ void gemm_body(const GemmArgs &g, double *smem, int tile_r, int tile_c)
 {
     constexpr int WGM = BM / 64, WGN = BN / 64;
@@ -331,6 +338,37 @@
             __builtin_amdgcn_sched_barrier(0);
         }
     }
+    if constexpr (FOUR) {
+        auto extra = [&](double *Cd, size_t ldd, double ad) {
+#pragma unroll
+            for (int i = 0; i < 4; ++i) {
+                double old[4][4];
+#pragma unroll
+                for (int r = 0; r < 4; ++r) {
+                    const int n = col0 + wn * 64 + i * 16 + 4 * r + l4;
+#pragma unroll
+                    for (int j = 0; j < 4; ++j) {
+                        const int m = row0 + wm * 64 + j * 16 + l15;
+                        old[r][j] = (interior || (m < g.m && n < g.n)) ? Cd[(size_t)m + (size_t)n * ldd] : 0.0;
+                    }
+                }
+                __builtin_amdgcn_sched_barrier(0);
+#pragma unroll
+                for (int r = 0; r < 4; ++r) {
+                    const int n = col0 + wn * 64 + i * 16 + 4 * r + l4;
+#pragma unroll
+                    for (int j = 0; j < 4; ++j) {
+                        const int m = row0 + wm * 64 + j * 16 + l15;
+                        if (interior || (m < g.m && n < g.n)) Cd[(size_t)m + (size_t)n * ldd] = __builtin_fma(ad, acc[i][j][r], old[r][j]);
+                    }
+                }
+                __builtin_amdgcn_sched_barrier(0);
+            }
+        };
+        extra(g.C2, g.ldc2, g.alpha2);
+        if (g.ndst > 2) extra(g.C3, g.ldc3, g.alpha3);
+        if (g.ndst > 3) extra(g.C4, g.ldc4, g.alpha4);
+    }
 }
 
 __device__ __forceinline__ unsigned lds_addr(const void *p)
@@ -358,7 +396,7 @@
 }
 #define SGPR_LGKM_WAIT(n) do { asm volatile("s_waitcnt lgkmcnt(" #n ")" ::: "memory"); __builtin_amdgcn_sched_barrier(0); } while (0)
 
-template <int BM, int BN, int STAGES, bool TWO = false>
+template <int BM, int BN, int STAGES, bool TWO = false, bool FOUR = false>
 __device__ __forceinline__ void gemm_body_dma(const GemmArgs &g, double *smem, int tile_r, int tile_c)
 {
     constexpr int WGM = BM / 64, WGN = BN / 64;
@@ -557,8 +595,37 @@
             __builtin_amdgcn_sched_barrier(0);
         }
     }
-}
-
-
-}
-}
+    if constexpr (FOUR) {
+        auto extra = [&](double *Cd, size_t ldd, double ad) {
+            double *const cb = Cd + (size_t)(row0 + wm * 64 + l15) + (size_t)(col0 + wn * 64 + l4) * ldd;
+            auto fetchd = [&](int i, double (&o)[4][4]) {
+#pragma unroll
+                for (int r = 0; r < 4; ++r)
+#pragma unroll
+                    for (int j = 0; j < 4; ++j) o[r][j] = cb[(size_t)(j * 16) + (size_t)(i * 16 + 4 * r) * ldd];
+            };
+            fetchd(0, old[0]);
+#pragma unroll
+            for (int i = 0; i < 4; ++i) {
+                if (i + 1 < 4) fetchd(i + 1, old[(i + 1) & 1]);
+                __builtin_amdgcn_sched_barrier(0);
+                if (i + 1 < 4) asm volatile("s_waitcnt vmcnt(16)" ::: "memory");
+                else           asm volatile("s_waitcnt vmcnt(0)" ::: "memory");
+                __builtin_amdgcn_sched_barrier(0);
+#pragma unroll
+                for (int r = 0; r < 4; ++r)
+#pragma unroll
+                    for (int j = 0; j < 4; ++j)
+                        cb[(size_t)(j * 16) + (size_t)(i * 16 + 4 * r) * ldd] = __builtin_fma(ad, acc[i][j][r], old[i & 1][r][j]);
+                __builtin_amdgcn_sched_barrier(0);
+            }
+        };
+        extra(g.C2, g.ldc2, g.alpha2);
+        if (g.ndst > 2) extra(g.C3, g.ldc3, g.alpha3);
+        if (g.ndst > 3) extra(g.C4, g.ldc4, g.alpha4);
+    }
+}
+
+
+}
+}
diff --git a/sympgpr_amd/csrc/probe.hip b/sympgpr_amd/csrc/probe.hip
--- a/sympgpr_amd/csrc/probe.hip
+++ b/sympgpr_amd/csrc/probe.hip
@@ -523,6 +523,22 @@
 {
     return gemm_nt_two(m, n, k, alpha, A, lda, B, ldb, beta, C, ldc, alpha2, C2, ldc2, static_cast<hipStream_t>(stream));
 }
+extern "C" int sgpr_probe_strassen2_plan(int m, int n, int k, int lower, long smin, long kslab, long smin2, long kslab2,
+                                         long scratch_doubles, long long *out, int max_records, int *count)
+{
+    if (!count || scratch_doubles < 0) { set_error("probe_strassen2_plan: bad arguments"); return SGPR_E_ARG; }
+    std::vector<long long> plan;
+    const int rc = strassen_outer_plan(m, n, k, lower, smin, kslab, smin2, kslab2, (size_t)scratch_doubles, plan);
+    if (rc) return rc;
+    *count = (int)(plan.size() / STRASSEN_REC);
+    for (size_t i = 0; out && i < plan.size() && (int)(i / STRASSEN_REC) < max_records; ++i) out[i] = plan[i];
+    return 0;
+}
+extern "C" int sgpr_probe_gemm_nt4_dev(int m, int n, int k, const double *A, size_t lda, const double *B, size_t ldb, double beta,
+                                       int count, double *const *C, const size_t *ldc, const double *alpha, void *stream)
+{
+    return gemm_nt_multi(m, n, k, A, lda, B, ldb, beta, count, C, ldc, alpha, static_cast<hipStream_t>(stream));
+}
 extern "C" unsigned sgpr_probe_map_calls(void) { return applymap_last_calls(); }
 extern "C" int sgpr_probe_map_team(int ntest, int n0) { return applymap_team(ntest, n0); }
 extern "C" int sgpr_probe_trsm_piece(int ticket, int cap, int strips, int out[5]) { if (ticket < 0 || cap < 1 || strips < 0 || !out) return SGPR_E_ARG; trsm_piece_of(ticket, cap, strips, out); return 0; }
```

Result: faster. 78.89, median of 6 (+3.4%).
